# iqbal-lab-org/gramtools

Measured on AMD Instinct MI355X. Metric: 150bp reads quasimapped/sec (whole node); bit-exact coverage, higher is better.
Workload: dtype u32

## Files before the change

### gramtools_amd/_lib.py

```python
import ctypes as C
import os

from .build import LIB, build_library


class GmxError(RuntimeError):
    def __init__(self, code, msg):
        super().__init__(f"gmx error {code}: {msg}")
        self.code = code


class IndexInfo(C.Structure):
    _fields_ = [("n_text", C.c_uint64), ("kmer_size", C.c_uint32), ("n_sites", C.c_uint32), ("is_nested", C.c_uint32),
                ("n_allele_slots", C.c_uint32), ("n_per_base_slots", C.c_uint32), ("n_grouped_slots", C.c_uint32),
                ("n_nodes", C.c_uint32), ("n_kmers_present", C.c_uint64), ("index_bytes", C.c_uint64),
                ("kmer_size2", C.c_uint32), ("n_inline_sites", C.c_uint32), ("seed_shift", C.c_uint32),
                ("n_jump_sites", C.c_uint32), ("n_seed_words", C.c_uint64)]


class EngineOpts(C.Structure):
    _fields_ = [("device", C.c_int), ("rng_mode", C.c_int), ("max_states", C.c_uint32),
                ("max_path_nodes", C.c_uint32), ("max_batch_reads", C.c_uint64), ("forward_only", C.c_int),
                ("huge_heap_bytes", C.c_uint64), ("log_cap_words", C.c_uint64)]


class Stats(C.Structure):
    _fields_ = [("all_reads_count", C.c_uint64), ("skipped_reads_count", C.c_uint64),
                ("missing_kmer_reads_count", C.c_uint64), ("no_extension_reads_count", C.c_uint64),
                ("exact_mapped_reads_count", C.c_uint64)]


class QueueCounts(C.Structure):
    _fields_ = [(n, C.c_uint64) for n in ("mapped", "alive", "dead", "overflow_probe", "overflow_extend", "big_mapped",
                                          "cover_general", "cover_mid", "cover_overflow", "seed_cursor", "huge_search",
                                          "inst_mapped", "huge_cover", "log_replays", "log_replayed_entries", "overflow_split")]


class StockReport(C.Structure):
    _fields_ = [(n, C.c_uint64) for n in ("kmers", "states", "kmer_mismatches", "kmers_missing_in_files", "duplicate_kmers",
                                          "mask_bits", "mask_mismatches", "cov_graph_state", "cov_graph_library_version",
                                          "cov_graph_sites", "fm_index_bytes")]


class Timing(C.Structure):
    _fields_ = [("search_ms", C.c_double), ("search_launches", C.c_uint64), ("cover_ms", C.c_double),
                ("cover_launches", C.c_uint64), ("reads", C.c_uint64), ("kernel_ms", C.c_double * 8),
                ("kernel_launches", C.c_uint64 * 8)]


class BgzfMember(C.Structure):
    _fields_ = [("offset", C.c_uint64), ("size", C.c_uint32), ("isize", C.c_uint32), ("crc32", C.c_uint32), ("reserved", C.c_uint32)]


class IngestResult(C.Structure):
    _fields_ = [("status", C.c_uint32), ("bad_member", C.c_uint32), ("n_reads", C.c_uint64), ("n_bases", C.c_uint64),
                ("n_pairs", C.c_uint64), ("uniform_len", C.c_uint32), ("any_skip", C.c_uint32), ("text_bytes", C.c_uint64),
                ("consumed_bytes", C.c_uint64), ("tail_bytes", C.c_uint64), ("sub_pairs", C.c_uint64 * 16),
                ("d_planes", C.c_void_p), ("d_offsets", C.c_void_p), ("d_skip", C.c_void_p)]


class DepthStats(C.Structure):
    _fields_ = [("mean_cov_depth", C.c_double), ("variance_cov_depth", C.c_double), ("num_sites_noCov", C.c_uint64),
                ("num_sites_total", C.c_uint64)]


class DeviceCoverage(C.Structure):
    _fields_ = [("allele_sum", C.c_void_p), ("n_allele_sum", C.c_uint64), ("per_base", C.c_void_p),
                ("n_per_base", C.c_uint64), ("grouped", C.c_void_p), ("n_grouped", C.c_uint64),
                ("stats", C.c_void_p), ("n_stats", C.c_uint64), ("fused", C.c_void_p), ("n_fused", C.c_uint64)]


_vp, _u64, _u32, _i64 = C.c_void_p, C.c_uint64, C.c_uint32, C.c_int64
_u8p, _u32p, _i32p, _u64p, _i64p = (C.POINTER(C.c_uint8), C.POINTER(C.c_uint32), C.POINTER(C.c_int32),
                                    C.POINTER(C.c_uint64), C.POINTER(C.c_int64))
SYMBOLS = {
    "gmx_last_error": (C.c_char_p, []),
    "gmx_index_build": (C.c_int, [_u32p, _u64, _u32, C.c_int, C.POINTER(_vp)]),
    "gmx_index_build_from_file": (C.c_int, [C.c_char_p, _u32, C.c_int, C.POINTER(_vp)]),
    "gmx_index_save": (C.c_int, [_vp, C.c_char_p]),
    "gmx_index_load": (C.c_int, [C.c_char_p, C.c_char_p, _u32, C.POINTER(_vp)]),
    "gmx_index_destroy": (None, [_vp]),
    "gmx_index_get_info": (C.c_int, [_vp, C.POINTER(IndexInfo)]),
    "gmx_index_site_layout": (C.c_int, [_vp, _u32p, _u32p, _u32p, _u32p, _i32p]),
    "gmx_index_per_base_layout": (_i64, [_vp, _u32p, _u64]),
    "gmx_index_allele_base_layout": (C.c_int, [_vp, _u32p, _u32p]),
    "gmx_compute_coverage_depth": (C.c_int, [_vp, _u32p, _u32p, _u32p, _u64, C.POINTER(DepthStats)]),
    "gmx_index_bubble_order": (C.c_int, [_vp, _u32p]),
    "gmx_debug_suffix_array_u16": (C.c_int, [C.POINTER(C.c_uint16), _u64, C.POINTER(C.c_uint16)]),
    "gmx_index_copy_sa": (C.c_int, [_vp, _u32p]),
    "gmx_index_copy_bwt": (C.c_int, [_vp, _u32p]),
    "gmx_index_rank": (_u32, [_vp, _u32, _u32]),
    "gmx_index_copy_pos_info": (C.c_int, [_vp, _i64p]),
    "gmx_index_copy_target_map": (_i64, [_vp, _i64p, _u64]),
    "gmx_index_seed_states": (_i64, [_vp, _u8p, _i64p, _u64]),
    "gmx_index_seed_states_k": (_i64, [_vp, _u8p, _u32, _i64p, _u64]),
    "gmx_index_jump_states": (_i64, [_vp, _u32, _u32, _i64p, _u64]),
    "gmx_engine_default_opts": (None, [C.POINTER(EngineOpts)]),
    "gmx_engine_create": (C.c_int, [_vp, C.POINTER(EngineOpts), C.POINTER(_vp)]),
    "gmx_engine_destroy": (None, [_vp]),
    "gmx_engine_reset": (C.c_int, [_vp]),
    "gmx_engine_reset_async": (C.c_int, [_vp, _vp]),
    "gmx_map_reads_host": (C.c_int, [_vp, _u8p, _u64p, _u32p, _u64]),
    "gmx_map_reads_device": (C.c_int, [_vp, _vp, _vp, _vp, _u64, _u64, _vp]),
    "gmx_map_reads_packed_host": (C.c_int, [_vp, _vp, _vp, _u32, _vp, _vp, _u64]),
    "gmx_engine_sync_uploads": (C.c_int, [_vp]),
    "gmx_engine_seeds_in_place": (C.c_int, [_vp, C.c_int]),
    "gmx_packed_pairs": (_u64, [_u64p, _u32, _u64]),
    "gmx_twobit_units": (_u64, [_u64p, _u32, _u64]),
    "gmx_pack_reads_2bit": (C.c_int, [_vp, _vp, _u32, _u64, _vp, _vp, C.c_int]),
    "gmx_map_reads_2bit_host": (C.c_int, [_vp, _vp, _vp, _u32, _vp, _vp, _u64]),
    "gmx_map_reads_packed_device": (C.c_int, [_vp, _vp, _vp, _u32, _vp, _vp, _u64]),
    "gmx_ingest_create": (C.c_int, [C.c_int, _u64, C.POINTER(_vp)]),
    "gmx_ingest_destroy": (None, [_vp]),
    "gmx_ingest_max_text": (_u64, [_vp]),
    "gmx_ingest_max_compressed": (_u64, [_vp]),
    "gmx_ingest_reset": (C.c_int, [_vp]),
    "gmx_ingest_set_format": (C.c_int, [_vp, C.c_int]),
    "gmx_ingest_set_bam_header": (C.c_int, [_vp, _u64]),
    "gmx_ingest_bam_rewalks": (_i64, [_vp]),
    "gmx_ingest_submit_bgzf": (C.c_int, [_vp, C.c_int, _vp, _u64, C.POINTER(BgzfMember), _u64, C.c_int]),
    "gmx_ingest_submit_text": (C.c_int, [_vp, C.c_int, _vp, _u64, C.c_int]),
    "gmx_ingest_submit_gzip": (C.c_int, [_vp, C.c_int, _vp, _u64, _u64, C.c_int]),
    "gmx_ingest_gzip_repairs": (_i64, [_vp]),
    "gmx_ingest_submit_text_deferred": (C.c_int, [_vp, C.c_int, _vp, _u64]),
    "gmx_ingest_max_members": (_u64, [_vp]),
    "gmx_ingest_wait": (C.c_int, [_vp, C.c_int, C.POINTER(IngestResult)]),
    "gmx_ingest_submit_bgzf_deferred": (C.c_int, [_vp, C.c_int, _vp, _u64, C.POINTER(BgzfMember), _u64]),
    "gmx_ingest_scan": (C.c_int, [_vp, C.c_int, _vp, _u64, C.c_int]),
    "gmx_ingest_fetch_tail": (_i64, [_vp, C.c_int, _vp, _u64]),
    "gmx_ingest_release_after": (C.c_int, [_vp, C.c_int, _vp]),
    "gmx_ingest_fetch_text": (_i64, [_vp, C.c_int, _vp, _u64]),
    "gmx_ingest_fetch_reads": (C.c_int, [_vp, C.c_int, _vp, _vp, _vp]),
    "gmx_pack_reads": (C.c_int, [_vp, _vp, _u32, _u64, _vp, _vp, C.c_int]),
    "gmx_engine_reserve": (C.c_int, [_vp, _u64, _u64]),
    "gmx_engine_reserve_packed": (C.c_int, [_vp, _u64, _u64]),
    "gmx_host_alloc": (_vp, [_u64]),
    "gmx_host_free": (None, [_vp]),
    "gmx_engine_sync": (C.c_int, [_vp]),
    "gmx_engine_enable_timing": (C.c_int, [_vp, C.c_int]),
    "gmx_engine_timing": (C.c_int, [_vp, C.POINTER(Timing)]),
    "gmx_engine_queue_counts": (C.c_int, [_vp, C.POINTER(QueueCounts)]),
    "gmx_stock_read_int_vector": (_i64, [C.c_char_p, _u32, _u64p, _u64, C.POINTER(C.c_uint32)]),
    "gmx_stock_write_int_vector": (C.c_int, [C.c_char_p, _u64p, _u64, _u32, C.c_int]),
    "gmx_index_write_stock_files": (C.c_int, [_vp, C.c_char_p]),
    "gmx_index_check_stock_files": (C.c_int, [_vp, C.c_char_p, C.POINTER(StockReport)]),
    "gmx_engine_second_stream": (_vp, [_vp]),
    "gmx_engine_debug_keep_states": (C.c_int, [_vp, C.c_int]),
    "gmx_debug_fail_alloc": (C.c_uint64, [C.c_int64]),
    "gmx_debug_final_states": (C.c_int, [_vp, _u64, _u32p, _u64, _u64p, C.POINTER(C.c_int)]),
    "gmx_debug_search": (C.c_int, [_vp, _u8p, _u32, C.c_int, _u32p, _u64, _u32, _u32, C.c_int, _u32p, _u64, _u64p]),
    "gmx_debug_encapsulate": (C.c_int, [_vp, _u32p, _u64, _u32p, _u64, _u64p, _u32p, _u64, _u64p]),
    "gmx_master_seeds": (C.c_int, [_u32, _u64p, _u64, _u32p]),
    "gmx_coverage_device": (C.c_int, [_vp, C.POINTER(DeviceCoverage)]),
    "gmx_coverage_reduce_begin": (C.c_int, [_vp, _vp]),
    "gmx_coverage_reduce_end": (C.c_int, [_vp, _vp]),
    "gmx_coverage_fetch": (C.c_int, [_vp, _u32p, _u32p, _u32p, C.POINTER(Stats)]),
    "gmx_coverage_fetch_grouped_log": (_i64, [_vp, _u32p, _u64]),
    "gmx_engine_record_outcomes": (C.c_int, [_vp, C.c_int]),
    "gmx_engine_outcome_count": (_i64, [_vp]),
    "gmx_engine_fetch_outcomes": (C.c_int, [_vp, _u64, _u64, _u8p]),
    "gmx_engine_record_positions": (C.c_int, [_vp, C.c_int]),
    "gmx_engine_position_count": (_i64, [_vp]),
    "gmx_engine_fetch_positions": (C.c_int, [_vp, _u64, _u64, _u32p]),
    "gmx_engine_record_strands": (C.c_int, [_vp, C.c_int]),
    "gmx_engine_set_max_candidates": (C.c_int, [_vp, C.c_uint32]),
    "gmx_engine_max_candidates": (C.c_uint32, [_vp]),
    "gmx_coverage_fetch_strand": (C.c_int, [_vp, C.c_int, _u32p, _u32p, _u32p]),
    "gmx_coverage_fetch_grouped_log_strand": (_i64, [_vp, C.c_int, _u32p, _u64]),
    "gmx_coverage_export_grouped_log": (_i64, [_vp, _u32p, _u64]),
    "gmx_coverage_import_grouped_log": (C.c_int, [_vp, _u32p, _u64, C.c_int]),
    "gmx_grouped_log_merge_gathered": (_i64, [_vp, _vp, C.c_int, _u64, _vp, _u64]),
# ... 66 lines not shown
```

### gramtools_amd/csrc/gmx_capi.cpp

```cpp
#include <atomic>
#include <algorithm>
#include <array>
#include <cmath>
#include <cstdlib>
#include <cstring>
#include <map>
#include <new>
#include <stdexcept>
#include <system_error>
#include <string>
#include <thread>
#include <vector>

#include "gmx_core.h"
#include "gmx_internal.h"

static std::atomic<uint64_t> g_index_serial{1};
struct gmx_index {
  gmx::HostIndex h;
  const uint64_t serial = g_index_serial.fetch_add(1);
};

static thread_local std::string g_error;
void gmx_set_error(const std::string &msg) noexcept {
// ... 320 lines not shown
      uint32_t nm = (1u << site.n_alleles) - 1u;
      for (uint32_t m = 0; m < nm; ++m) {
        uint32_t tot = grouped_raw[h.l_grouped_off[s] + m];
        if (!tot) continue;
        uint16_t c = (uint16_t)(tot & 0xFFFFu);
        for (uint32_t a = 0; a < site.n_alleles; ++a)
          if (((m + 1) >> a) & 1u) hap[s][(int32_t)a] = (uint16_t)(hap[s][(int32_t)a] + c);
      }
    }
    for (auto &e : logged[s])
      for (auto a : e.first) hap[s][a] = (uint16_t)(hap[s][a] + e.second);
  }
  auto max_hap = [&](size_t s) -> std::pair<int32_t, uint16_t> {
    std::pair<int32_t, uint16_t> best{0, 0};
    bool any = false;
    for (auto &e : hap[s])
      if (!any || e.second > best.second) {
        best = {e.first, e.second};
        any = true;
      }
    return best;
  };
  std::vector<double> coverages;
  double total = 0;
  uint64_t no_cov = 0;
  for (uint32_t s : bubble_order(h)) {
    const GmxSite &site = h.sites[s];
    if (site.parent_site != 0) continue;
    auto mx = max_hap(s);
    uint16_t allele_cov = mx.second;
    double sum = 0;
    uint64_t n_bases = 0;
    uint32_t cur = site.entry_node;
    size_t guard = 0;
    while (cur != site.exit_node) {
      if (++guard > h.nodes.size() + 8) {
        gmx_set_error("coverage graph walk does not terminate");
        return GMX_EINVAL;
      }
      const GmxNode &nd = h.nodes[cur];
      uint32_t ne = h.nodes[cur + 1].edge_begin - nd.edge_begin;
      if (ne > 1 && nd.seq_len == 0) {
        auto m2 = max_hap((nd.site - 5) / 2);
        if (m2.first < 0 || (uint32_t)m2.first >= ne) {
          gmx_set_error("haplogroup out of range");
          return GMX_EINVAL;
        }
        cur = h.edges[nd.edge_begin + (uint32_t)m2.first];
        continue;
      }
      if (nd.seq_len > 0 && nd.cov_off != GMX_NO_COV)
        for (uint32_t i = 0; i < nd.seq_len; ++i) {
          uint32_t v = per_base_raw[h.l_cov_off[cur] + i];
          sum += (double)(v > 65535u ? 65535u : v);
          ++n_bases;
        }
      cur = h.edges[nd.edge_begin];
    }
    double site_cov = n_bases ? sum / (double)n_bases : (double)allele_cov;
    total += site_cov;
    coverages.push_back(site_cov);
    if (allele_cov == 0) no_cov++;
  }
  double mean = total / (double)coverages.size();
  double tv = 0;
  for (double c : coverages) tv += std::pow(c - mean, 2);
  out->mean_cov_depth = mean;
  out->variance_cov_depth = tv / (double)coverages.size();
  out->num_sites_noCov = no_cov;
  out->num_sites_total = coverages.size();
  return GMX_OK;
} GMX_GUARD_INT("gmx_compute_coverage_depth")

int gmx_debug_suffix_array_u16(const uint16_t *text, uint64_t n, uint16_t *out) try {
  try {
    gmx::debug_suffix_array_u16(text, (size_t)n, out);
    return GMX_OK;
  } catch (std::exception const &ex) {
    gmx_set_error(ex.what());
    return GMX_EINVAL;
  }
} GMX_GUARD_INT("gmx_debug_suffix_array_u16")

int gmx_index_copy_sa(const gmx_index *ix, uint32_t *out) try {
  memcpy(out, ix->h.sa.data(), ix->h.sa.size() * 4);
  return GMX_OK;
} GMX_GUARD_INT("gmx_index_copy_sa")
int gmx_index_copy_bwt(const gmx_index *ix, uint32_t *out) try {
  if (ix->h.bwt.empty()) {
    gmx_set_error("this index was built without its introspection tables (GMX_INDEX_INTROSPECTION=1 keeps them)");
    return GMX_EINVAL;
  }
  memcpy(out, ix->h.bwt.data(), ix->h.bwt.size() * 4);
  return GMX_OK;
} GMX_GUARD_INT("gmx_index_copy_bwt")
uint32_t gmx_index_rank(const gmx_index *ix, uint32_t upper, uint32_t base) try {
  if (base < 1 || base > 4) return 0;
  GmxIndexView v = ix->h.view();
  return gmx_rank(v, upper, base);
} GMX_GUARD_ZERO("gmx_index_rank")
int gmx_index_copy_pos_info(const gmx_index *ix, int64_t *out) try {
  const auto &h = ix->h;
  if (h.pos_target.size() != h.prg.size()) {
    gmx_set_error("this index was built without its introspection tables (GMX_INDEX_INTROSPECTION=1 keeps them)");
    return GMX_EINVAL;
  }
  for (size_t p = 0; p < h.prg.size(); ++p) {
    const GmxNode &nd = h.nodes[h.pos_node[p]];
    out[5 * p + 0] = nd.site;
    out[5 * p + 1] = nd.allele;
    out[5 * p + 2] = h.prg[p] <= 4 ? (int64_t)p - nd.first_pos : 0;
    out[5 * p + 3] = h.pos_target[p].first;
    out[5 * p + 4] = h.pos_target[p].second;
  }
  return GMX_OK;
} GMX_GUARD_INT("gmx_index_copy_pos_info")
int64_t gmx_index_copy_target_map(const gmx_index *ix, int64_t *out, uint64_t cap) try {
  std::vector<int64_t> v{(int64_t)ix->h.target_map.size()};
  for (auto &e : ix->h.target_map) {
    v.push_back(e.first);
    v.push_back((int64_t)e.second.size());
    for (auto &t : e.second) {
      v.push_back(t.id);
      v.push_back(t.deletion_allele);
    }
  }
  if (v.size() > cap) return -(int64_t)v.size();
  std::copy(v.begin(), v.end(), out);
  return (int64_t)v.size();
} GMX_GUARD_INT("gmx_index_copy_target_map")
int64_t gmx_index_seed_states(const gmx_index *ix, const uint8_t *kmer, int64_t *out, uint64_t cap) try {
  return gmx_index_seed_states_k(ix, kmer, ix->h.kmer_size, out, cap);
} GMX_GUARD_INT("gmx_index_seed_states")
int64_t gmx_index_seed_states_k(const gmx_index *ix, const uint8_t *kmer, uint32_t len, int64_t *out, uint64_t cap) try {
  const auto &h = ix->h;
  if (len == 0 || (len != h.kmer_size && len != h.kmer_size2)) return GMX_EINVAL;
  uint32_t code = 0;
  for (uint32_t j = 0; j < len; ++j) {
    if (kmer[j] < 1 || kmer[j] > 4) return GMX_EINVAL;
    code |= (uint32_t)(kmer[j] - 1) << (2 * j);
  }
  auto v = gmx::seed_states_of(h, code, len != h.kmer_size);
  if (v.size() > cap) return -(int64_t)v.size();
  std::copy(v.begin(), v.end(), out);
  return (int64_t)v.size();
} GMX_GUARD_INT("gmx_index_seed_states_k")
int64_t gmx_index_jump_states(const gmx_index *ix, uint32_t lo, uint32_t hi, int64_t *out, uint64_t cap) try {
  const auto &h = ix->h;
  GmxIndexView v = h.view();
  ProbeCtx ctx;
  const GmxRankBlock b = v.blocks[lo >> GMX_BLK_SHIFT];
  gmx_marker_pass(v, lo, hi, GMX_NIL, GMX_NIL, b, ctx);
  std::vector<int64_t> r{(int64_t)ctx.n};
  for (uint32_t s = 0; s < ctx.n; ++s) {
    r.push_back(ctx.st[s].lo);
    r.push_back(ctx.st[s].hi);
    std::vector<std::pair<uint32_t, int32_t>> tmp;
    for (uint32_t x = ctx.st[s].tvd; x != GMX_NIL; x = ctx.arena[x].next) tmp.push_back({ctx.arena[x].site, ctx.arena[x].allele});
    r.push_back((int64_t)tmp.size());
    for (size_t i = tmp.size(); i-- > 0;) {
      r.push_back(tmp[i].first);
      r.push_back(tmp[i].second);
    }
    tmp.clear();
    for (uint32_t x = ctx.st[s].tvg; x != GMX_NIL; x = ctx.arena[x].next) tmp.push_back({ctx.arena[x].site, -1});
    r.push_back((int64_t)tmp.size());
// ... 231 lines not shown
```

### gramtools_amd/csrc/gmx_engine_cover_kernels.h

```cpp
#pragma once
struct CoverAcc {
  uint32_t *acc;
  uint32_t *log;
  uint32_t *log_cursor;
  uint32_t log_cap;
  uint32_t *scratch_big;
  uint32_t n_lanes_big;
  int rng_mode;
  uint32_t max_candidates;
  uint32_t log_sites;
  uint32_t *heap;
  uint64_t heap_words;
  const uint32_t *status;
  uint32_t n_tasks;
  unsigned long long *stats;
  uint32_t rev_off;
  __device__ __forceinline__ uint32_t off_of(uint32_t task) const { return (task & 1u) ? rev_off : 0u; }
};

#define GMX_LOG_PAD 0xFFFFFFFFu
#ifdef GMX_LOOP_STATS
__device__ unsigned long long gmx_cover_stats[6 * 16];
__device__ unsigned long long gmx_coop_stats[6 * 8];
extern "C" int gmx_debug_coop_stats(unsigned long long *out, int reset) {
// ... 787 lines not shown

template <bool NESTED>
__global__ void __launch_bounds__(GMX_BLOCK) gmx_cover_single_kernel(GmxIndexView ix, BatchView b, SearchOut o, CoverAcc acc) {
  const uint32_t region = blockIdx.x & (GMX_REGIONS - 1);
  const uint32_t n_mapped = o.counters[(16 + region) * GMX_CNT_STRIDE];
  const uint32_t m = (blockIdx.x / GMX_REGIONS) * GMX_BLOCK + threadIdx.x;
  if (m >= n_mapped) return;
  gmx_cover_single_rec<NESTED>(ix, o, acc, (size_t)region * o.region_cap + m, o.cover_general_list, 8u);
}

struct StageLds {
  uint32_t *w;
  __device__ __forceinline__ uint32_t cap() const { return GMX_STAGE_MAX; }
  __device__ __forceinline__ void put(uint32_t i, uint32_t v) { w[i * GMX_BLOCK] = v; }
  __device__ __forceinline__ uint32_t get(uint32_t i) const { return w[i * GMX_BLOCK]; }
};
#ifndef GMX_JUMP_MIN_BLOCKS
#define GMX_JUMP_MIN_BLOCKS 1
#endif
__global__ void __launch_bounds__(GMX_BLOCK, GMX_JUMP_MIN_BLOCKS) gmx_cover_jump_kernel(GmxIndexView ix, BatchView b, SearchOut o, CoverAcc acc) {
  const uint32_t region = blockIdx.x & (GMX_REGIONS - 1);
  const uint32_t n_mapped = o.counters[(16 + region) * GMX_CNT_STRIDE];
  const uint32_t m = (blockIdx.x / GMX_REGIONS) * GMX_BLOCK + threadIdx.x;
  if (m >= n_mapped) return;
  const size_t rec_idx = (size_t)region * o.region_cap + m;
  CompactEnv env;
  env.rec = o.cover_recs[rec_idx];
  env.acc = acc.acc;
  env.acc_off = acc.rev_off ? acc.off_of(o.cover_rec_task[rec_idx]) : 0u;
  env.log = nullptr;
  env.log_cursor = nullptr;
  env.log_cap = 0;
  env.log_sites = 0;
  env.status = GMX_TASK_MAPPED;
  env.log_at = env.log_end = 0;
  const uint32_t p = env.rec.p, tvd = env.n_trav() ? 0u : GMX_NIL, tvg = env.rec.tvg;
  StageLds stage{gmx_lds + threadIdx.x};
  const bool done = gmx_cover_jump(ix, env, stage, p, tvd, tvg, env.rec.len_n & 0xFFFFu);
  if (!done) o.single_rest_list[atomicAdd(&o.counters[GMX_CNT_SINGLE_REST * GMX_CNT_STRIDE], 1u)] = (uint32_t)rec_idx;
}
__global__ void __launch_bounds__(GMX_BLOCK) gmx_cover_single_rest_kernel(GmxIndexView ix, BatchView b, SearchOut o, CoverAcc acc) {
  const uint32_t n = o.counters[GMX_CNT_SINGLE_REST * GMX_CNT_STRIDE];
  for (uint32_t i = blockIdx.x * GMX_BLOCK + threadIdx.x; i < n; i += gridDim.x * GMX_BLOCK)
    gmx_cover_single_rec<false>(ix, o, acc, o.single_rest_list[i], o.cover_general_list, 8u);
}

__global__ void gmx_log_replay_setup_kernel(SearchOut o, const uint32_t *retry_huge_in) {
  uint32_t *c = o.counters;
  const uint32_t n_entries = c[GMX_CNT_LOG_RETRY * GMX_CNT_STRIDE], n_recs = c[GMX_CNT_LOG_RETRY_RECS * GMX_CNT_STRIDE],
                 n_huge = c[GMX_CNT_LOG_RETRY_HUGE * GMX_CNT_STRIDE];
  for (uint32_t i = threadIdx.x; i < n_huge; i += blockDim.x) o.huge_list[i] = retry_huge_in[i];
  __syncthreads();
  if (threadIdx.x == 0) {
    c[4 * GMX_CNT_STRIDE] = n_entries;
    c[GMX_CNT_REPLAY_RECS * GMX_CNT_STRIDE] = n_recs;
    c[11 * GMX_CNT_STRIDE] = n_huge;
    c[15 * GMX_CNT_STRIDE] = 0;
    c[14 * GMX_CNT_STRIDE] = 0;
    c[GMX_CNT_LOG_RETRY * GMX_CNT_STRIDE] = 0;
    c[GMX_CNT_LOG_RETRY_RECS * GMX_CNT_STRIDE] = 0;
    c[GMX_CNT_LOG_RETRY_HUGE * GMX_CNT_STRIDE] = 0;
  }
}
template <bool NESTED>
__global__ void __launch_bounds__(GMX_BLOCK) gmx_cover_single_replay_kernel(GmxIndexView ix, BatchView b, SearchOut o, CoverAcc acc,
                                                                            const uint32_t *recs_in) {
  const uint32_t n = o.counters[GMX_CNT_REPLAY_RECS * GMX_CNT_STRIDE];
  for (uint32_t i = blockIdx.x * GMX_BLOCK + threadIdx.x; i < n; i += gridDim.x * GMX_BLOCK)
    gmx_cover_single_rec<NESTED>(ix, o, acc, recs_in[i], o.cover_overflow_list, 4u);
}

__global__ void gmx_stats_limbs_kernel(unsigned long long *stats, uint32_t *limbs, int recombine) {
  const uint32_t t = threadIdx.x;
  if (!recombine) {
    if (t < 20) limbs[t] = (uint32_t)((stats[t >> 2] >> (16 * (t & 3))) & 0xFFFFull);
    else if (t < 32) limbs[t] = 0;
  } else if (t < 5) {
    unsigned long long v = 0;
    for (int l = 3; l >= 0; --l) v = (v << 16) + limbs[4 * t + l];
    stats[t] = v;
  }
}

#define GMX_PACK_READS 128
#define GMX_PACK_IN_BYTES (24 * 1024)
#define GMX_PACK_OUT_PAIRS (GMX_PACK_IN_BYTES / 32 + GMX_PACK_READS + 8)
typedef uint32_t __attribute__((aligned(1))) gmx_u32_unaligned;
__device__ __forceinline__ void pack4(uint32_t x, uint32_t &lo, uint32_t &hi, uint32_t &bad) {
  uint32_t y = x - 0x01010101u;
  bad |= ((y & ~x & 0x80808080u) | (y & 0xFCFCFCFCu));
  lo = (((y & 0x01010101u) * 0x01020408u) >> 24) & 0xFu;
  hi = ((((y >> 1) & 0x01010101u) * 0x01020408u) >> 24) & 0xFu;
}
__device__ __forceinline__ uint2 pack_tail(const uint8_t *p, uint32_t rem, uint32_t &bad) {
  uint2 out = make_uint2(0, 0);
  for (uint32_t j = 0; j < rem; ++j) {
    uint32_t x = p[j];
    if (x < 1 || x > 4) bad = 1;
    out.x |= ((x - 1u) & 1u) << j;
    out.y |= (((x - 1u) >> 1) & 1u) << j;
  }
  return out;
}
#define GMX_PACK_THREADS (2 * GMX_PACK_READS)
__global__ void __launch_bounds__(GMX_PACK_THREADS) gmx_pack_kernel(BatchView b, uint8_t *skip, uint2 *packed, uint32_t *counters,
                                                                    uint32_t *zero, uint32_t zero_words) {
  __shared__ uint4 in4[GMX_PACK_IN_BYTES / 16 + 2];
  __shared__ uint2 outp[GMX_PACK_OUT_PAIRS];
  if (blockIdx.x == 0)
    for (uint32_t i = threadIdx.x; i < GMX_N_COUNTERS * GMX_CNT_STRIDE; i += GMX_PACK_THREADS) counters[i] = 0;
  for (uint32_t i = blockIdx.x * GMX_PACK_THREADS + threadIdx.x; i < zero_words; i += gridDim.x * GMX_PACK_THREADS) zero[i] = 0;
  const uint32_t r0 = blockIdx.x * GMX_PACK_READS;
  const uint32_t r1 = min(r0 + GMX_PACK_READS, b.n_reads);
  const uint32_t read = r0 + (threadIdx.x >> 1), half = threadIdx.x & 1u;
  const uint64_t s0 = b.offsets[r0], s1 = b.offsets[r1];
  const uintptr_t g0 = reinterpret_cast<uintptr_t>(b.reads + s0);
  const uint32_t shift = (uint32_t)(g0 & 15u);
  const uint64_t span = (s1 - s0) + shift;
  if (span <= GMX_PACK_IN_BYTES) {
    const uint4 *src = reinterpret_cast<const uint4 *>(g0 - shift);
    const uint32_t n16 = (uint32_t)((span + 15) >> 4);
    {
      uint32_t i = threadIdx.x;
      for (; i + 2 * GMX_PACK_THREADS < n16; i += 3 * GMX_PACK_THREADS) {
        const uint4 v0 = src[i], v1 = src[i + GMX_PACK_THREADS], v2 = src[i + 2 * GMX_PACK_THREADS];
        in4[i] = v0;
        in4[i + GMX_PACK_THREADS] = v1;
        in4[i + 2 * GMX_PACK_THREADS] = v2;
      }
      for (; i < n16; i += GMX_PACK_THREADS) in4[i] = src[i];
    }
    const uint64_t po0 = pack_off(b, r0);
    const uint32_t n_out = (uint32_t)(pack_off(b, r1) - po0);
    for (uint32_t i = threadIdx.x; i < n_out; i += GMX_PACK_THREADS) outp[i] = make_uint2(0, 0);
    __syncthreads();
    if (read < r1) {
      const uint64_t s = b.offsets[read];
      const uint32_t len = (uint32_t)(b.offsets[read + 1] - s);
      const uint32_t q = shift + (uint32_t)(s - s0);
      const uint32_t *w = reinterpret_cast<const uint32_t *>(in4);
      const uint8_t *bytes = reinterpret_cast<const uint8_t *>(in4);
      uint2 *out = outp + (uint32_t)(pack_off(b, read) - po0);
      const uint32_t full = len >> 5, first_half = (full + 1u) >> 1;
      const uint32_t c0 = half ? first_half : 0u, c1 = half ? full : first_half;
      uint32_t idx = (q >> 2) + 8u * c0;
      const uint32_t sh = q & 3u;
      uint32_t bad = 0;
      uint32_t carry = w[idx];
      for (uint32_t c = c0; c < c1; ++c) {
        uint2 pair = make_uint2(0, 0);
#pragma unroll
        for (int j = 0; j < 8; ++j) {
          uint32_t nxt = w[++idx], lo, hi;
          pack4(__builtin_amdgcn_alignbyte(nxt, carry, sh), lo, hi, bad);
          pair.x |= lo << (4 * j);
          pair.y |= hi << (4 * j);
          carry = nxt;
        }
        out[c] = pair;
      }
      const uint32_t rem = len & 31u;
      if (half && rem) out[full] = pack_tail(bytes + q + full * 32, rem, bad);
      bad |= (uint32_t)__shfl_xor((int)bad, 1);
      if (!half) skip[read] = bad ? 1 : 0;
    }
    __syncthreads();
// ... 26 lines not shown
```

### gramtools_amd/csrc/gmx_engine_debug.h

```cpp

struct GmxDebugPools {
  GmxFinalState *states = nullptr;
  uint32_t *stack = nullptr;
  GmxPathNode *arena = nullptr;
  uint32_t *result = nullptr;
  uint32_t *in = nullptr;
  uint2 *planes = nullptr;
  uint32_t cap_states = 0, cap_nodes = 0, cap_in = 0, cap_pairs = 0;
};

__global__ void __launch_bounds__(64) gmx_debug_search_kernel(GmxIndexView ix, BatchView b, const uint32_t *in, uint32_t from, uint32_t stop,
                                                              uint32_t mode, uint32_t from_seed_table, BigOut g, uint32_t *result) {
  const bool active = threadIdx.x == 0;
  BigCtx ctx;
  ctx.sp = 0;
  ctx.cap = g.max_states;
  ctx.stack = g.stack;
  ctx.arena = g.arena;
  ctx.arena_n = 0;
  ctx.arena_cap = g.max_path_nodes;
  ctx.status = GMX_TASK_MAPPED;
  ctx.out = g.states;
  ctx.n_out = 0;
  ctx.out_cap = g.max_states;
// ... 92 lines not shown
  for (uint32_t h = st.traversed; h != GMX_NIL;) {
    GmxPathNode nd;
    int rc = node(h, nd);
    if (rc) return rc;
    tvd.emplace_back(nd.site, nd.allele);
    h = nd.next;
    if (tvd.size() > (1u << 20)) {
      gmx_set_error("debug states: path list does not end");
      return GMX_EREF;
    }
  }
  for (uint32_t h = st.traversing; h != GMX_NIL;) {
    if (gmx_h_inline(h)) {
      tvg.push_back(5u + 2u * (h & ~GMX_INLINE_FLAG));
      break;
    }
    GmxPathNode nd;
    int rc = node(h, nd);
    if (rc) return rc;
    tvg.push_back(nd.site);
    h = nd.next;
    if (tvg.size() > (1u << 20)) {
      gmx_set_error("debug states: path list does not end");
      return GMX_EREF;
    }
  }
  w.put(lo);
  w.put(hi);
  w.put((uint32_t)tvd.size());
  w.put((uint32_t)tvg.size());
  for (size_t i = tvd.size(); i-- > 0;) {
    w.put(tvd[i].first);
    w.put((uint32_t)tvd[i].second);
  }
  for (size_t i = tvg.size(); i-- > 0;) w.put(tvg[i]);
  return GMX_OK;
}

int debug_pools(gmx_engine *e, GmxDebugPools &p, uint32_t n_in_words, uint32_t n_pairs) {
  const uint32_t S = std::max<uint32_t>(e->big.max_states, 64u), N = std::max<uint32_t>(e->big.max_path_nodes, 64u);
  int rc;
  if ((rc = e->alloc(&p.states, S, false))) return rc;
  if ((rc = e->alloc(&p.stack, (size_t)S * GMX_STACK_WORDS, false))) return rc;
  if ((rc = e->alloc(&p.arena, N, false))) return rc;
  if ((rc = e->alloc(&p.result, 4, true))) return rc;
  if ((rc = e->alloc(&p.in, std::max<uint32_t>(n_in_words, 1u), false))) return rc;
  if ((rc = e->alloc(&p.planes, n_pairs + 16, true))) return rc;
  p.cap_states = S;
  p.cap_nodes = N;
  return GMX_OK;
}
void debug_pools_free(gmx_engine *e, GmxDebugPools &p) {
  e->release(p.states);
  e->release(p.stack);
  e->release(p.arena);
  e->release(p.result);
  e->release(p.in);
  e->release(p.planes);
}

}

extern "C" {

int gmx_engine_debug_keep_states(gmx_engine *e, int on) try {
  if (!e) {
    gmx_set_error("null engine");
    return GMX_EINVAL;
  }
  e->keep_states = on != 0;
  return GMX_OK;
} GMX_GUARD_INT("gmx_engine_debug_keep_states")

int gmx_debug_final_states(gmx_engine *e, uint64_t task, uint32_t *out, uint64_t cap_words, uint64_t *n_words, int *tier) try {
  if (!e || !n_words) {
    gmx_set_error("gmx_debug_final_states: null argument");
    return GMX_EINVAL;
  }
  if (!e->keep_states || task >= 2 * e->keep_reads) {
    gmx_set_error("gmx_debug_final_states: no such task in the last batch (gmx_engine_debug_keep_states first)");
    return GMX_EINVAL;
  }
  HIP_TRY(hipSetDevice(e->opts.device));
  HIP_TRY(hipDeviceSynchronize());
  int rc = debug_isa(e);
  if (rc) return rc;
  uint32_t raw[GMX_N_COUNTERS * GMX_CNT_STRIDE];
  HIP_TRY(hipMemcpy(raw, e->d_counters, sizeof(raw), hipMemcpyDeviceToHost));
  auto c = [&](int i) { return raw[i * GMX_CNT_STRIDE]; };
  DebugWriter w{out, cap_words};
  {
    const uint32_t n_huge = c(11);
    std::vector<uint32_t> huge(n_huge);
    if (n_huge) HIP_TRY(hipMemcpy(huge.data(), e->d_huge, n_huge * sizeof(uint32_t), hipMemcpyDeviceToHost));
    for (uint32_t t : huge)
      if (t == task) {
        gmx_set_error("gmx_debug_final_states: the task was searched by the last tier, which keeps no states");
        return GMX_ECAP;
      }
  }
  const uint32_t used = (uint32_t)std::min<uint64_t>((uint64_t)c(1) + c(9) + c(29), e->big.max_slots);
  if (used) {
    std::vector<uint32_t> owner(used), nf(used), over(std::min<uint32_t>(c(1), used));
    HIP_TRY(hipMemcpy(owner.data(), e->big.task_of_slot, used * sizeof(uint32_t), hipMemcpyDeviceToHost));
    HIP_TRY(hipMemcpy(nf.data(), e->big.n_final, used * sizeof(uint32_t), hipMemcpyDeviceToHost));
    if (!over.empty()) HIP_TRY(hipMemcpy(over.data(), e->d_overflow, over.size() * sizeof(uint32_t), hipMemcpyDeviceToHost));
    bool in_slots = false;
    for (uint32_t s = used; s-- > 0;) {
      const bool first_q = s < over.size();
      if (first_q && (over[s] & ~GMX_INST_FLAG) != task) continue;
      if (!first_q && owner[s] != task) continue;
      in_slots = true;
      if (first_q && owner[s] != task) continue;
      if (nf[s] == 0) continue;
      const bool inst = first_q && (over[s] & GMX_INST_FLAG) != 0;
      const uint32_t n = nf[s];
      std::vector<GmxFinalState> st(n);
      if (inst) {
        uint32_t first = 0, width = 0;
        HIP_TRY(hipMemcpy(&first, e->d_inst_first + s, 4, hipMemcpyDeviceToHost));
        HIP_TRY(hipMemcpy(&width, e->d_inst_width + s, 4, hipMemcpyDeviceToHost));
        if (n > width * GMX_INST_STATES) continue;
        HIP_TRY(hipMemcpy(st.data(), e->d_inst_states + (size_t)first * GMX_INST_STATES, n * sizeof(GmxFinalState), hipMemcpyDeviceToHost));
        const GmxPathNode *arena = e->d_inst_arena + (size_t)first * GMX_FAST_ARENA;
        w.put(n);
        for (uint32_t i = 0; i < n; ++i) {
          rc = debug_put_state(e, w, st[i], [&](uint32_t h, GmxPathNode &nd) {
            HIP_TRY(hipMemcpy(&nd, arena + h, sizeof(nd), hipMemcpyDeviceToHost));
            return GMX_OK;
          });
          if (rc) return rc;
        }
        if (tier) *tier = 2;
      } else {
        if (n > e->big.max_states) continue;
        HIP_TRY(hipMemcpy(st.data(), e->big.states + (size_t)s * e->big.max_states, n * sizeof(GmxFinalState), hipMemcpyDeviceToHost));
        const GmxPathNode *arena = e->big.arena + (size_t)s * e->big.max_path_nodes;
        w.put(n);
        for (uint32_t i = 0; i < n; ++i) {
          rc = debug_put_state(e, w, st[i], [&](uint32_t h, GmxPathNode &nd) {
            HIP_TRY(hipMemcpy(&nd, arena + h, sizeof(nd), hipMemcpyDeviceToHost));
            return GMX_OK;
          });
          if (rc) return rc;
        }
        if (tier) *tier = 1;
      }
      *n_words = w.n;
      return w.n > cap_words && out ? GMX_ECAP : GMX_OK;
    }
    if (in_slots) {
      w.put(0);
      if (tier) *tier = 1;
      *n_words = w.n;
      return GMX_OK;
    }
  }
  uint32_t packed = 0;
  HIP_TRY(hipMemcpy(&packed, e->d_n_final + task, 4, hipMemcpyDeviceToHost));
  const uint32_t n = std::min<uint32_t>(packed & 0xFFu, GMX_FAST_STATES);
  std::vector<GmxFinalState> st(n);
  if (n) HIP_TRY(hipMemcpy(st.data(), e->d_finals + (size_t)task * GMX_FAST_STATES, n * sizeof(GmxFinalState), hipMemcpyDeviceToHost));
  const GmxPathNode *arena = e->d_arena + task;
  w.put(n);
  for (uint32_t i = 0; i < n; ++i) {
    rc = debug_put_state(e, w, st[i], [&](uint32_t h, GmxPathNode &nd) {
      HIP_TRY(hipMemcpy(&nd, arena + h, sizeof(nd), hipMemcpyDeviceToHost));
      return GMX_OK;
    });
    if (rc) return rc;
  }
  if (tier) *tier = 0;
  *n_words = w.n;
  return w.n > cap_words && out ? GMX_ECAP : GMX_OK;
} GMX_GUARD_INT("gmx_debug_final_states")

int gmx_debug_search(gmx_engine *e, const uint8_t *read, uint32_t read_len, int from_seed_table, const uint32_t *states, uint64_t n_state_words,
                     uint32_t from, uint32_t stop, int lf_only, uint32_t *out, uint64_t cap_words, uint64_t *n_words) try {
  if (!e || !read || !n_words || read_len == 0 || (!from_seed_table && (!states || n_state_words == 0 || from > read_len || stop > from))) {
    gmx_set_error("gmx_debug_search: bad argument");
    return GMX_EINVAL;
  }
  for (uint32_t i = 0; i < read_len; ++i)
    if (read[i] < 1 || read[i] > 4) {
      gmx_set_error("gmx_debug_search: the read must hold bases 1..4");
      return GMX_EINVAL;
    }
  if (from_seed_table && read_len < e->dview.kmer_size) {
    gmx_set_error("gmx_debug_search: read shorter than the k-mer size");
    return GMX_EINVAL;
  }
  HIP_TRY(hipSetDevice(e->opts.device));
  HIP_TRY(hipDeviceSynchronize());
  int rc = debug_isa(e);
  if (rc) return rc;
  const uint32_t n_pairs = (read_len + 31u) / 32u;
  GmxDebugPools p;
  if ((rc = debug_pools(e, p, (uint32_t)n_state_words, n_pairs))) return rc;
  std::vector<uint2> planes(n_pairs + 16, make_uint2(0, 0));
  for (uint32_t i = 0; i < read_len; ++i) {
    const uint32_t code = read[i] - 1u;
    planes[i >> 5].x |= (code & 1u) << (i & 31u);
    planes[i >> 5].y |= (code >> 1) << (i & 31u);
  }
  HIP_TRY(hipMemcpy(p.planes, planes.data(), planes.size() * sizeof(uint2), hipMemcpyHostToDevice));
  if (!from_seed_table) HIP_TRY(hipMemcpy(p.in, states, n_state_words * sizeof(uint32_t), hipMemcpyHostToDevice));
  BatchView b{};
  b.packed = p.planes;
  b.n_reads = 1;
  b.forward_only = 1;
  b.uniform_len = read_len;
  b.pairs_per_read = n_pairs;
  BigOut g{};
  g.states = p.states;
  g.stack = p.stack;
  g.arena = p.arena;
  g.max_states = p.cap_states;
  g.max_path_nodes = p.cap_nodes;
  g.max_slots = 1;
  const size_t big_lds = (size_t)GMX_BIG_LDS_DEPTH * GMX_STACK_WORDS * 64 * sizeof(uint32_t);
  hipLaunchKernelGGL(gmx_debug_search_kernel, dim3(1), dim3(64), big_lds, 0, e->dview, b, p.in, from, stop,
                     lf_only ? GMX_MODE_LF : GMX_MODE_STATE, from_seed_table ? 1u : 0u, g, p.result);
  HIP_TRY(hipGetLastError());
  HIP_TRY(hipDeviceSynchronize());
  uint32_t res[3] = {0, 0, 0};
  HIP_TRY(hipMemcpy(res, p.result, sizeof(res), hipMemcpyDeviceToHost));
  if (res[0] != GMX_TASK_MAPPED) {
    debug_pools_free(e, p);
    gmx_set_error(res[0] == GMX_TASK_OVERFLOW ? "gmx_debug_search: the states exceed the engine's large-capacity pools (gmx_engine_opts.max_states / max_path_nodes)"
                                              : "gmx_debug_search: the search reports a condition on which the reference throws");
    return res[0] == GMX_TASK_OVERFLOW ? GMX_ECAP : GMX_EREF;
  }
  const uint32_t n = res[1];
  std::vector<GmxFinalState> st(n);
  std::vector<GmxPathNode> arena(res[2]);
  if (n) HIP_TRY(hipMemcpy(st.data(), p.states, n * sizeof(GmxFinalState), hipMemcpyDeviceToHost));
  if (res[2]) HIP_TRY(hipMemcpy(arena.data(), p.arena, res[2] * sizeof(GmxPathNode), hipMemcpyDeviceToHost));
  debug_pools_free(e, p);
  DebugWriter w{out, cap_words};
  w.put(n);
  for (uint32_t i = 0; i < n; ++i) {
    rc = debug_put_state(e, w, st[i], [&](uint32_t h, GmxPathNode &nd) {
      if (h >= arena.size()) {
        gmx_set_error("gmx_debug_search: path handle outside the arena");
        return GMX_EREF;
      }
      nd = arena[h];
      return GMX_OK;
    });
    if (rc) return rc;
  }
  *n_words = w.n;
  return w.n > cap_words && out ? GMX_ECAP : GMX_OK;
} GMX_GUARD_INT("gmx_debug_search")

int gmx_debug_encapsulate(gmx_engine *e, const uint32_t *states, uint64_t n_state_words, uint32_t *out, uint64_t cap_words, uint64_t *n_words,
                          uint32_t *nonvariant_sa, uint64_t cap_nonvariant, uint64_t *n_nonvariant) try {
  if (!e || !states || n_state_words == 0 || !n_words || !n_nonvariant) {
    gmx_set_error("gmx_debug_encapsulate: bad argument");
    return GMX_EINVAL;
  }
  HIP_TRY(hipSetDevice(e->opts.device));
  HIP_TRY(hipDeviceSynchronize());
  std::vector<GmxFinalState> st;
  std::vector<GmxPathNode> arena;
  const uint32_t *p = states, *end = states + n_state_words;
  const uint32_t ns = *p++;
  uint64_t positions = 0;
  for (uint32_t s = 0; s < ns; ++s) {
    if (p + 4 > end || p + 4 + 2 * (uint64_t)p[2] + p[3] > end) {
      gmx_set_error("gmx_debug_encapsulate: malformed state words");
      return GMX_EINVAL;
    }
    const uint32_t lo = p[0], hi = p[1], nt = p[2], ng = p[3];
    p += 4;
    if (lo > hi || hi >= e->dview.n) {
      gmx_set_error("gmx_debug_encapsulate: interval outside the suffix array");
      return GMX_EINVAL;
    }
    uint32_t tvd = GMX_NIL, tvg = GMX_NIL;
    for (uint32_t j = 0; j < nt; ++j, p += 2) {
      arena.push_back(GmxPathNode{p[0], (int32_t)p[1], tvd});
      tvd = (uint32_t)arena.size() - 1;
    }
    for (uint32_t j = 0; j < ng; ++j, ++p) {
      arena.push_back(GmxPathNode{p[0], -1, tvg});
      tvg = (uint32_t)arena.size() - 1;
    }
    st.push_back(GmxFinalState{lo, hi, tvd, tvg});
    positions += (uint64_t)hi - lo + 1;
  }
  if (positions > (1u << 24)) {
    gmx_set_error("gmx_debug_encapsulate: more than 2^24 positions");
    return GMX_EINVAL;
  }
  const uint32_t cap_items = (uint32_t)std::max<uint64_t>(positions + ns, 1);
  GmxFinalState *d_st = nullptr;
  uint32_t *d_out = nullptr;
  int rc;
  if ((rc = e->alloc(&d_st, st.size(), false))) return rc;
  if ((rc = e->alloc(&d_out, 2 + 7 * (size_t)cap_items, true))) return rc;
  if (!st.empty()) HIP_TRY(hipMemcpy(d_st, st.data(), st.size() * sizeof(GmxFinalState), hipMemcpyHostToDevice));
  hipLaunchKernelGGL(gmx_debug_items_kernel, dim3(1), dim3(64), 0, 0, e->dview, d_st, (uint32_t)st.size(), d_out, cap_items);
  HIP_TRY(hipGetLastError());
  HIP_TRY(hipDeviceSynchronize());
  std::vector<uint32_t> res(2 + 7 * (size_t)cap_items);
  HIP_TRY(hipMemcpy(res.data(), d_out, res.size() * sizeof(uint32_t), hipMemcpyDeviceToHost));
  e->release(d_st);
  e->release(d_out);
  if (res[0] == 0xFFFFFFFFu || res[1] > cap_items) {
    gmx_set_error("gmx_debug_encapsulate: item buffer exceeded");
    return GMX_EREF;
  }
  DebugWriter w{out, cap_words};
  w.put(res[0]);
  for (uint32_t i = 0; i < res[0]; ++i) {
    const uint32_t *it = res.data() + 2 + 6 * (size_t)i;
    GmxFinalState f{it[0], it[1], it[2], it[3]};
    if (it[4] != 0) {
      w.put(f.lo);
      w.put(f.lo);
      w.put(1);
      w.put(0);
      w.put(it[4]);
      w.put(it[5]);
      continue;
    }
    rc = debug_put_state(e, w, f, [&](uint32_t h, GmxPathNode &nd) {
      if (h >= arena.size()) {
        gmx_set_error("gmx_debug_encapsulate: path handle outside the arena");
        return GMX_EREF;
      }
      nd = arena[h];
      return GMX_OK;
    });
    if (rc) return rc;
  }
  *n_words = w.n;
  *n_nonvariant = res[1];
  for (uint32_t i = 0; i < res[1] && nonvariant_sa && i < cap_nonvariant; ++i) nonvariant_sa[i] = res[2 + 6 * (size_t)cap_items + i];
  return (w.n > cap_words && out) || (nonvariant_sa && res[1] > cap_nonvariant) ? GMX_ECAP : GMX_OK;
} GMX_GUARD_INT("gmx_debug_encapsulate")

}
```

### gramtools_amd/csrc/gmx_engine_host.h

```cpp
#pragma once
#define HIP_TRY(expr)                                                                      \
  do {                                                                                     \
    hipError_t _e = (expr);                                                                \
    if (_e != hipSuccess) {                                                                \
      gmx_set_error(std::string(#expr) + ": " + hipGetErrorString(_e));                    \
      return GMX_EHIP;                                                                     \
    }                                                                                      \
  } while (0)

enum : int { GMX_TK_SEED = 0, GMX_TK_FILTER0, GMX_TK_FILTER1, GMX_TK_SINGLE, GMX_TK_EXTEND2, GMX_TK_UNPACK, GMX_TK_N };
static_assert(GMX_TK_N <= GMX_TIMED_KERNELS, "gmx_timing::kernel_ms holds GMX_TIMED_KERNELS entries");

struct GmxReadLog {
  const uint32_t stride;
  bool on = false;
  uint32_t *d = nullptr;
  uint64_t cap = 0, count = 0;

  uint64_t used() const { return (count * stride + 3) & ~3ull; }

  int reserve(uint64_t n_more) {
    const uint64_t need = (count + n_more) * stride;
    if (need <= cap) return GMX_OK;
    const uint64_t grown = (std::max<uint64_t>(need + need / 2, 1u << 20) + 3) & ~3ull;
// ... 72 lines not shown
  GmxFinalState *d_inst_states = nullptr;
  uint32_t *d_inst_first = nullptr, *d_inst_width = nullptr;
  uint32_t *d_inst_serial = nullptr, *d_general_serial = nullptr, *d_big_serial = nullptr, *d_overflow3 = nullptr;
  bool coop = true;
  uint32_t *d_heap = nullptr;
  uint64_t heap_words = 0;
  bool log_sites = false;
  std::map<std::vector<uint32_t>, std::array<uint64_t, 2>> log_counts;
  uint32_t *h_log_state = nullptr;
  hipEvent_t ev_log_state = nullptr;
  bool log_state_pending = false;
  uint32_t *d_log_retry[2] = {nullptr, nullptr}, *d_log_retry_recs[2] = {nullptr, nullptr}, *d_log_retry_huge[2] = {nullptr, nullptr};
  int log_retry_side = 0;
  BatchView last_b{};
  SearchOut last_o{};
  CoverAcc last_acc{};
  size_t last_big_lds = 0;
  uint64_t log_replays = 0, log_replayed_entries = 0;
  uint64_t log_known = 0;
  uint64_t log_reads_since = 0;
  bool reset_pending = false;
  hipStream_t reset_stream = nullptr;
  hipStream_t side2_stream = nullptr;
  hipEvent_t ev_fork2 = nullptr, ev_side1 = nullptr, ev_filter = nullptr;
  hipStream_t side_stream = nullptr;
  hipEvent_t ev_fork = nullptr, ev_join = nullptr;
  hipEvent_t ev_wait = nullptr;
  struct GmxDeviceIndex *shared_index = nullptr;
  uint32_t filter_lds_words = 0;
  const uint32_t *d_kmer_planar = nullptr;
  const uint32_t *d_absent = nullptr;
  uint32_t n_absent = 0;
  bool use_absent = false;
  uint32_t n_cus = 256;
  uint32_t probe_iters = GMX_PROBE_ITERS;
  uint32_t extend_cap = 0;
  uint32_t extend_budget = 8;
  bool seeds_in_place = false;
  gmx_engine *twin = nullptr;
  gmx_engine *owner = nullptr;
  bool is_twin = false, twin_off = false;
  GmxReadLog outcomes{1}, positions{16};
  uint64_t reset_epoch = 0;
  hipStream_t main_stream = nullptr;
  uint32_t twin_toggle = 0;
  hipEvent_t ev_zeroed = nullptr, ev_twin_done = nullptr;
  uint64_t zero_epoch = 0, seen_zero_epoch = 0;
  bool twin_in_flight = false;
  bool last_on_twin = false;
  uint32_t extend_passes = 1;
  uint32_t extend_budget2[GMX_EXTRA_PASSES] = {24, 96, 0};
  GmxParked *d_park2 = nullptr;
  uint32_t *d_park2_n = nullptr;
  bool keep_states = false;
  uint64_t keep_reads = 0;
  std::vector<uint32_t> debug_isa;
  uint32_t fuse = 1;
  uint8_t *d_reads = nullptr;
  uint64_t *d_offsets = nullptr;
  uint32_t *d_seeds = nullptr;
  uint64_t cap_bases = 0, cap_stage_reads = 0;
  struct StageSlot {
    uint8_t *d_reads = nullptr;
    uint64_t *d_offsets = nullptr, *h_offsets = nullptr;
    uint32_t *d_seeds = nullptr, *h_seeds = nullptr;
    uint64_t cap_bases = 0, cap_reads = 0;
    hipEvent_t copied = nullptr, done = nullptr;
    bool busy = false;
  } stage[2];
  hipStream_t copy_stream = nullptr;
  hipStream_t copy_stream2 = nullptr;
  uint32_t copy_toggle = 0;
  hipStream_t last_stream = nullptr;
  struct PackSlot {
    uint2 *d_planes = nullptr;
    uint64_t *d_offsets = nullptr;
    uint32_t *d_seeds = nullptr;
    uint8_t *d_skip = nullptr;
    uint64_t cap_pairs = 0, cap_reads = 0;
    hipEvent_t copied = nullptr, done = nullptr;
    bool busy = false;
  } pslot[3];
  uint32_t pslot_next = 0;
  void release(void *q) {
    if (!q) return;
    for (size_t i = 0; i < allocs.size(); ++i)
      if (allocs[i] == q) {
        allocs[i] = allocs.back();
        allocs.pop_back();
        (void)hipFree(q);
        return;
      }
  }
  bool timing = false;
  struct EvTriple { hipEvent_t s, a, b, c; uint64_t reads; hipEvent_t k[GMX_TIMED_KERNELS][2]; uint32_t timed; };
  std::vector<EvTriple> pending;
  double search_ms = 0, cover_ms = 0;
  uint64_t search_launches = 0, cover_launches = 0, timed_reads = 0;
  double kernel_ms[GMX_TIMED_KERNELS] = {0};
  uint64_t kernel_launches[GMX_TIMED_KERNELS] = {0};

  template <class T>
  int alloc(T **p, size_t count, bool zero) {
    void *q = nullptr;
    size_t bytes = std::max<size_t>(count, 1) * sizeof(T);
    allocs.reserve(allocs.size() + 1);
    HIP_TRY(hipMalloc(&q, bytes));
    if (zero) HIP_TRY(hipMemset(q, 0, bytes));
    allocs.push_back(q);
    *p = (T *)q;
    return GMX_OK;
  }
  template <class T, class A>
  int upload(const T **dst, const std::vector<T, A> &src) {
    T *q = nullptr;
    int rc = alloc(&q, src.size(), false);
    if (rc) return rc;
    if (!src.empty()) HIP_TRY(hipMemcpy(q, src.data(), src.size() * sizeof(T), hipMemcpyHostToDevice));
    index_bytes += src.size() * sizeof(T);
    *dst = q;
    return GMX_OK;
  }
  int upload(const uint32_t **dst, const gmx::WordBuf &src) {
    uint32_t *q = nullptr;
    int rc = alloc(&q, src.size(), false);
    if (rc) return rc;
    const size_t piece = (size_t)1 << 28;
    for (size_t at = 0; at < src.size(); at += piece)
      HIP_TRY(hipMemcpy(q + at, src.data() + at, std::min(piece, src.size() - at) * sizeof(uint32_t), hipMemcpyHostToDevice));
    index_bytes += src.size() * sizeof(uint32_t);
    *dst = q;
    return GMX_OK;
  }
};

static hipError_t gmx_event_wait(hipEvent_t ev) {
  static const bool spin = getenv("GMX_WAIT_SPIN") != nullptr;
  if (spin) return hipEventSynchronize(ev);
  const auto t0 = std::chrono::steady_clock::now();
  for (bool napping = false;;) {
    const hipError_t q = hipEventQuery(ev);
    if (q != hipErrorNotReady) return q;
    (void)hipGetLastError();
    if (!napping) {
      napping = std::chrono::steady_clock::now() - t0 > std::chrono::microseconds(60);
      continue;
    }
    struct timespec ts = {0, 50 * 1000};
    nanosleep(&ts, nullptr);
  }
}

static int gmx_quiesce(gmx_engine *e) {
  if (!e->ev_wait) HIP_TRY(hipEventCreateWithFlags(&e->ev_wait, hipEventDisableTiming | hipEventBlockingSync));
  hipStream_t streams[5] = {e->last_stream, e->copy_stream, e->side_stream, e->side2_stream, e->copy_stream2};
  for (int i = 0; i < 5; ++i) {
    if (i > 0 && !streams[i]) continue;
    bool seen = false;
    for (int j = 0; j < i; ++j) seen = seen || streams[j] == streams[i];
    if (seen) continue;
    HIP_TRY(hipEventRecord(e->ev_wait, streams[i]));
    HIP_TRY(gmx_event_wait(e->ev_wait));
  }
  return GMX_OK;
}

static int note_zeroed(gmx_engine *e, hipStream_t stream) {
  if (!e->twin) return GMX_OK;
  if (!e->ev_zeroed) HIP_TRY(hipEventCreateWithFlags(&e->ev_zeroed, hipEventDisableTiming));
  HIP_TRY(hipEventRecord(e->ev_zeroed, stream));
  ++e->zero_epoch;
  return GMX_OK;
}
static int twin_join(gmx_engine *e, hipStream_t stream) {
  gmx_engine *tw = e->twin;
  if (!tw || !e->twin_in_flight) return GMX_OK;
  if (!e->ev_twin_done) HIP_TRY(hipEventCreateWithFlags(&e->ev_twin_done, hipEventDisableTiming));
  HIP_TRY(hipEventRecord(e->ev_twin_done, tw->main_stream));
  HIP_TRY(hipStreamWaitEvent(stream, e->ev_twin_done, 0));
  return GMX_OK;
}
static int flush_reset(gmx_engine *e) {
  if (!e->reset_pending) return GMX_OK;
  e->reset_pending = false;
  HIP_TRY(hipMemsetAsync(e->d_fused, 0, (e->n_fused + 32) * 4, e->reset_stream));
  return note_zeroed(e, e->reset_stream);
}

static int log_settle(gmx_engine *e);
static int gmx_log_drain(gmx_engine *e, uint64_t keep_below) {
  int frc = flush_reset(e);
  if (frc) return frc;
  HIP_TRY(hipDeviceSynchronize());
  uint32_t used = 0;
  HIP_TRY(hipMemcpy(&used, e->d_log_cursor, 4, hipMemcpyDeviceToHost));
  used = std::min(used, e->log_cap);
  e->log_reads_since = 0;
  e->log_known = used;
  if (used <= keep_below) return GMX_OK;
  std::vector<uint32_t> w(used);
  HIP_TRY(hipMemcpy(w.data(), e->d_log, (size_t)used * 4, hipMemcpyDeviceToHost));
  std::vector<uint32_t> key;
  for (size_t i = 0; i < w.size();) {
    if (w[i] == GMX_LOG_PAD) {
      ++i;
      continue;
    }
    const size_t n_ids = i + 2 > w.size() ? 0 : (size_t)(w[i + 1] & ~GMX_LOG_REVERSE);
    if (i + 2 > w.size() || i + 2 + n_ids > w.size()) {
      gmx_set_error("grouped-allele-count log: malformed record at word " + std::to_string(i) + " of " + std::to_string(w.size()));
      return GMX_EREF;
    }
    if ((w[i + 1] & GMX_LOG_REVERSE) && !(e->owner ? e->owner : e)->record_strands) {
      gmx_set_error("grouped-allele-count log: a reverse-complement record at word " + std::to_string(i) + " of an engine that does not record per strand");
      return GMX_EREF;
    }
    key.assign(1, w[i]);
    key.insert(key.end(), w.begin() + i + 2, w.begin() + i + 2 + n_ids);
    e->log_counts[key][(w[i + 1] & GMX_LOG_REVERSE) ? 1 : 0] += 1;
    i += 2 + n_ids;
  }
  HIP_TRY(hipMemset(e->d_log_cursor, 0, 4));
  e->log_known = 0;
  return GMX_OK;
}

template <class Env, int LIST>
static void launch_cover_lds(gmx_engine *e, hipStream_t stream, const BatchView &b, const SearchOut &o, const CoverAcc &acc,
                             bool after_coop = false) {
  static const uint32_t lanes_env = getenv("GMX_COVER_LANES") ? (uint32_t)atoi(getenv("GMX_COVER_LANES")) : 0u;
  const uint32_t lanes = lanes_env ? std::min(lanes_env, gmx_cover_lds_lanes<Env>()) : gmx_cover_lds_lanes<Env>();
  const size_t lds = (size_t)GmxScratchFixed<Env>::total * lanes * sizeof(uint32_t);
  const uint32_t per_cu = std::min<uint32_t>((uint32_t)(160 * 1024 / lds), 32u);
  hipLaunchKernelGGL((gmx_cover_kernel<Env, LIST>), dim3(e->n_cus * per_cu), dim3(64), lds, stream, e->dview, b, o, e->big,
                     acc, lanes, after_coop ? 1u : 0u);
}

template <int LIST>
static void launch_cover_coop(gmx_engine *e, hipStream_t stream, const BatchView &b, const SearchOut &o, const CoverAcc &acc) {
  const size_t lds = (size_t)gmx_coop_lds_words<LIST>() * sizeof(uint32_t);
  const uint32_t per_cu = std::min<uint32_t>((uint32_t)(160 * 1024 / lds), 16u);
  hipLaunchKernelGGL((gmx_cover_coop_kernel<LIST>), dim3(e->n_cus * per_cu), dim3(64), lds, stream, e->dview, b, o, e->big, acc);
}

extern "C" {

void gmx_engine_default_opts(gmx_engine_opts *o) try {
  o->device = 0;
  o->rng_mode = GMX_RNG_LEMIRE;
  o->max_states = 1024;
  o->max_path_nodes = 2048;
  o->max_batch_reads = 4u << 20;
  o->forward_only = 0;
  o->huge_heap_bytes = 512ull << 20;
  o->log_cap_words = 0;
} GMX_GUARD_VOID("gmx_engine_default_opts")

static int ensure_batch_capacity(gmx_engine *e, uint64_t n_reads, bool launching = false) {
  if (launching) {
    gmx_engine *own = e->owner ? e->owner : e;
    for (GmxReadLog *log : {&own->outcomes, &own->positions})
      if (log->on) {
        const int lrc = log->reserve(n_reads);
        if (lrc) return lrc;
      }
  }
  if (n_reads <= e->cap_reads) return GMX_OK;
  uint64_t cap = std::max<uint64_t>(e->cap_reads ? n_reads + n_reads / 8 : n_reads, 1024);
  uint64_t n_tasks = cap * 2;
  int rc;
  if ((rc = e->alloc(&e->d_skip, cap, true))) return rc;
  if ((rc = e->alloc(&e->d_status, n_tasks, false))) return rc;
  if ((rc = e->alloc(&e->d_n_final, n_tasks, false))) return rc;
  if ((rc = e->alloc(&e->d_cover_recs, n_tasks * GMX_REGIONS, false))) return rc;
  if ((rc = e->alloc(&e->d_mapped, n_tasks * GMX_REGIONS, false))) return rc;
  if ((rc = e->alloc(&e->d_task_lists, (size_t)GMX_TL_N * n_tasks, false))) return rc;
  e->d_overflow = e->d_task_lists + (size_t)GMX_TL_OVERFLOW * n_tasks;
  e->d_overflow2 = e->d_task_lists + (size_t)GMX_TL_OVERFLOW2 * n_tasks;
  e->d_alive = e->d_task_lists + (size_t)GMX_TL_ALIVE * n_tasks;
  e->d_dead = e->d_task_lists + (size_t)GMX_TL_DEAD * n_tasks;
  e->d_dead2 = e->d_task_lists + (size_t)GMX_TL_DEAD2 * n_tasks;
  e->d_cover_general = e->d_task_lists + (size_t)GMX_TL_GENERAL * n_tasks;
  if ((rc = e->alloc(&e->d_cover_overflow, n_tasks, false))) return rc;
  if ((rc = e->alloc(&e->d_general_rest, n_tasks, false))) return rc;
  if ((rc = e->alloc(&e->d_single_rest, n_tasks, false))) return rc;
  if ((rc = e->alloc(&e->d_park2, (size_t)n_tasks * GMX_STACK_DEPTH, false))) return rc;
  if ((rc = e->alloc(&e->d_park2_n, n_tasks, false))) return rc;
  if (e->log_sites)
    for (int side = 0; side < 2; ++side) {
      if ((rc = e->alloc(&e->d_log_retry[side], n_tasks, false))) return rc;
      if ((rc = e->alloc(&e->d_log_retry_recs[side], n_tasks, false))) return rc;
      if ((rc = e->alloc(&e->d_log_retry_huge[side], n_tasks, false))) return rc;
    }
  if ((rc = e->alloc(&e->d_cover_mid, n_tasks, false))) return rc;
  if ((rc = e->alloc(&e->d_seed_cursor, n_tasks, false))) return rc;
  if ((rc = e->alloc(&e->d_finals, n_tasks * GMX_FAST_STATES, false))) return rc;
  if ((rc = e->alloc(&e->d_arena, n_tasks * GMX_FAST_ARENA, false))) return rc;
  if ((rc = e->alloc(&e->d_alive_seed, n_tasks, false))) return rc;
  if ((rc = e->alloc(&e->d_huge, n_tasks, false))) return rc;
  if ((rc = e->alloc(&e->d_cover_huge, n_tasks, false))) return rc;
  if ((rc = e->alloc(&e->d_huge_retry, 2 * n_tasks, false))) return rc;
  e->big.max_slots = (uint32_t)std::min<uint64_t>(n_tasks, std::min<uint64_t>(std::max<uint64_t>(n_tasks / 16, 4096), 262144));
  if ((rc = e->alloc(&e->big.states, (size_t)e->big.max_slots * e->big.max_states, false))) return rc;
  if ((rc = e->alloc(&e->big.stack, (size_t)e->big.max_slots * e->big.max_states * GMX_STACK_WORDS, false))) return rc;
  if ((rc = e->alloc(&e->big.arena, (size_t)e->big.max_slots * e->big.max_path_nodes, false))) return rc;
  if ((rc = e->alloc(&e->big.n_final, e->big.max_slots, false))) return rc;
  if ((rc = e->alloc(&e->big.task_of_slot, e->big.max_slots, false))) return rc;
  if ((rc = e->alloc(&e->d_big_mapped, e->big.max_slots, false))) return rc;
  e->inst_cap = (uint32_t)std::min<uint64_t>(n_tasks, 1u << 23);
  if ((rc = e->alloc(&e->d_inst_list, e->inst_cap, false))) return rc;
  if ((rc = e->alloc(&e->d_inst_sa, e->inst_cap, false))) return rc;
  if ((rc = e->alloc(&e->d_inst_remaining, e->big.max_slots, false))) return rc;
  if ((rc = e->alloc(&e->d_inst_mapped, e->big.max_slots, false))) return rc;
  if ((rc = e->alloc(&e->d_inst_first, e->big.max_slots, false))) return rc;
  if ((rc = e->alloc(&e->d_inst_width, e->big.max_slots, false))) return rc;
  if ((rc = e->alloc(&e->d_inst_serial, e->big.max_slots, false))) return rc;
  if ((rc = e->alloc(&e->d_general_serial, n_tasks, false))) return rc;
  if ((rc = e->alloc(&e->d_big_serial, e->big.max_slots, false))) return rc;
  if ((rc = e->alloc(&e->d_overflow3, 2 * n_tasks, false))) return rc;
  if ((rc = e->alloc(&e->d_inst_arena, (size_t)e->inst_cap * GMX_FAST_ARENA, false))) return rc;
  if ((rc = e->alloc(&e->d_inst_states, (size_t)e->inst_cap * GMX_INST_STATES, false))) return rc;
  e->cap_reads = cap;
  return GMX_OK;
}

struct GmxDeviceIndex {
  uint64_t serial = 0;
  int device = 0;
  GmxIndexView view{};
  std::vector<void *> allocs;
  uint64_t bytes = 0;
  int refs = 0;
};
static std::mutex g_dev_index_mu;
static std::vector<GmxDeviceIndex *> g_dev_indexes;
static void gmx_dev_index_release(GmxDeviceIndex *d) {
  if (!d) return;
  std::lock_guard<std::mutex> lk(g_dev_index_mu);
  if (--d->refs > 0) return;
  for (void *p : d->allocs) (void)hipFree(p);
  g_dev_indexes.erase(std::remove(g_dev_indexes.begin(), g_dev_indexes.end(), d), g_dev_indexes.end());
// ... 153 lines not shown
                   : e->log_sites     ? (1ull << 26)
                                      : 64;
    e->log_cap = (uint32_t)std::min<uint64_t>(cap, 0xFFFFFF00ull);
  }
  if (primary)
    e->d_log = primary->d_log;
  else
    rc |= e->alloc(&e->d_log, e->log_cap, false);
  e->heap_words = opts.huge_heap_bytes / 4 / 64 * 64;
  rc |= e->alloc(&e->d_heap, e->heap_words, false);
  rc |= e->alloc(&e->d_counters, GMX_N_COUNTERS * GMX_CNT_STRIDE, true);
  e->big.max_states = opts.max_states;
  e->big.max_path_nodes = opts.max_path_nodes;
  e->big.max_slots = 0;
  {
    hipDeviceProp_t prop;
    if (hipGetDeviceProperties(&prop, opts.device) == hipSuccess && prop.multiProcessorCount > 0)
      e->n_cus = (uint32_t)prop.multiProcessorCount;
    const size_t words = h.kmer_bitmap.size();
    if (!getenv("GMX_FORCE_ABSENT_FILTER") && words >= 4 && words % 4 == 0 && words * 4 <= 128 * 1024 &&
        hipFuncSetAttribute(reinterpret_cast<const void *>(gmx_filter_lds_kernel), hipFuncAttributeMaxDynamicSharedMemorySize,
                            (int)(words * 4)) == hipSuccess)
      e->filter_lds_words = (uint32_t)words;
    (void)hipGetLastError();
    if (primary) {
      e->filter_lds_words = primary->filter_lds_words;
      e->d_kmer_planar = primary->d_kmer_planar;
      e->d_absent = primary->d_absent;
      e->n_absent = primary->n_absent;
      e->use_absent = primary->use_absent;
    } else if (e->filter_lds_words) {
      const uint32_t k = h.kmer_size;
      std::vector<uint32_t> planar(words, 0);
      for (uint64_t code = 0; code < (1ull << (2 * k)); ++code) {
        if (!((h.kmer_bitmap[code >> 5] >> (code & 31)) & 1u)) continue;
        uint32_t lo = 0, hi = 0;
        for (uint32_t j = 0; j < k; ++j) {
          const uint32_t base = (uint32_t)(code >> (2 * j)) & 3u;
          lo |= (base & 1u) << j;
          hi |= (base >> 1) << j;
        }
        const uint32_t p = (hi << k) | lo;
        planar[p >> 5] |= 1u << (p & 31);
      }
      rc |= e->upload(&e->d_kmer_planar, planar);
    } else if (!getenv("GMX_NO_ABSENT_FILTER")) {
      const uint64_t n_k = 1ull << (2 * h.kmer_size);
      if (n_k - std::min<uint64_t>(n_k, h.n_seed_kmers_present) <= GMX_ABSENT_MAX) {
        std::vector<uint32_t> absent;
        for (size_t w = 0; w < words && absent.size() <= GMX_ABSENT_MAX; ++w) {
          uint32_t zeros = ~h.kmer_bitmap[w];
          while (zeros) {
            const uint64_t code = (uint64_t)w * 32 + (uint32_t)__builtin_ctz(zeros);
            zeros &= zeros - 1;
            if (code < n_k) absent.push_back((uint32_t)code);
          }
        }
        if (absent.size() <= GMX_ABSENT_MAX) {
          e->n_absent = (uint32_t)absent.size();
          e->use_absent = true;
          if (absent.empty()) absent.push_back(0);
          rc |= e->upload(&e->d_absent, absent);
        }
      }
    }
  }
  if (const char *pi = getenv("GMX_PROBE_ITERS")) e->probe_iters = (uint32_t)std::max(0, atoi(pi));
  if (getenv("GMX_NO_FUSE")) e->fuse = 0;
  if (const char *eb = getenv("GMX_EXTEND_BUDGET")) e->extend_budget = (uint32_t)std::max(0, atoi(eb));
  e->extend_cap = 0u;
  if (const char *ec = getenv("GMX_EXTEND_CAP")) e->extend_cap = (uint32_t)std::max(0, atoi(ec));
  e->extend_passes = 1u;
  e->extend_budget2[0] = 24;
  e->extend_budget2[1] = 96;
  if (const char *ep = getenv("GMX_EXTEND_PASSES")) {
    e->extend_passes = 1;
    for (const char *q = ep; *q && e->extend_passes < GMX_EXTRA_PASSES;) {
      e->extend_budget2[e->extend_passes - 1] = (uint32_t)std::max(1l, strtol(q, const_cast<char **>(&q), 10));
      ++e->extend_passes;
      if (*q == ',') ++q; else break;
    }
  }
  if (getenv("GMX_NO_COOP")) e->coop = false;
  e->seed_cursor = h.n_seed_states_large * 10 > h.n_seed_states;
  if (const char *sc = getenv("GMX_SEED_CURSOR")) e->seed_cursor = atoi(sc) != 0;
  if (primary) {
    e->seed_cursor = primary->seed_cursor;
    e->dview.sa_ctx = primary->dview.sa_ctx;
    e->dview.seed_side = primary->dview.seed_side;
  }
  if (!primary && e->seed_cursor && !rc && !getenv("GMX_NO_SA_CTX")) {
    uint32_t *sc = nullptr;
    if (e->alloc(&sc, h.sa.size(), false) == GMX_OK) {
      hipLaunchKernelGGL(gmx_sa_ctx_kernel, dim3(8192), dim3(256), 0, nullptr, e->dview.sa, e->dview.text, (uint64_t)h.sa.size(), sc);
      if (hipDeviceSynchronize() == hipSuccess) {
        e->dview.sa_ctx = sc;
        e->index_bytes += h.sa.size() * sizeof(uint32_t);
      }
    } else {
      (void)hipGetLastError();
    }
  }
  if (!primary && e->seed_cursor && !rc && !getenv("GMX_NO_SEED_SIDE") && h.seed_words.size() > 1) {
    uint32_t *side = nullptr;
    const size_t n_side = h.seed_words.size() / 4 + 2;
    if (e->alloc(&side, n_side, false) == GMX_OK) {
      hipLaunchKernelGGL(gmx_seed_side_kernel, dim3(8192), dim3(256), 0, nullptr, e->dview.seeds, (uint64_t)h.seeds.size(), e->dview.seed_words,
                         e->dview.seed_shift, side);
      if (h.kmer_size2)
        hipLaunchKernelGGL(gmx_seed_side_kernel, dim3(8192), dim3(256), 0, nullptr, e->dview.seeds2, (uint64_t)h.seeds2.size(), e->dview.seed_words,
                           e->dview.seed_shift, side);
      if (hipDeviceSynchronize() == hipSuccess) {
        e->dview.seed_side = side;
        e->index_bytes += n_side * sizeof(uint32_t);
      }
    } else {
      (void)hipGetLastError();
    }
  }
  auto make_stream = [&](hipStream_t *st) -> bool {
    int least = 0, greatest = 0;
    bool want_prio = h.is_nested;
    if (const char *tp = getenv("GMX_TWIN_PRIORITY")) want_prio = atoi(tp) != 0;
    const bool prio = primary && want_prio && hipDeviceGetStreamPriorityRange(&least, &greatest) == hipSuccess && least != greatest;
    (void)hipGetLastError();
    return (prio ? hipStreamCreateWithPriority(st, hipStreamNonBlocking, greatest) : hipStreamCreateWithFlags(st, hipStreamNonBlocking)) == hipSuccess;
  };
  rc |= !make_stream(&e->side_stream);
  rc |= !make_stream(&e->side2_stream);
  rc |= hipEventCreateWithFlags(&e->ev_fork2, hipEventDisableTiming) != hipSuccess;
  rc |= hipEventCreateWithFlags(&e->ev_side1, hipEventDisableTiming) != hipSuccess;
  rc |= hipEventCreateWithFlags(&e->ev_filter, hipEventDisableTiming) != hipSuccess;
  rc |= hipEventCreateWithFlags(&e->ev_fork, hipEventDisableTiming) != hipSuccess;
  rc |= hipEventCreateWithFlags(&e->ev_join, hipEventDisableTiming) != hipSuccess;
  e->cover_big_lanes = 64 * 32;
  rc |= e->alloc(&e->d_scratch_big, (size_t)GmxScratchFixed<CoverEnvBig>::total * e->cover_big_lanes, false);
  if (primary) {
    e->is_twin = true;
    rc |= !make_stream(&e->main_stream);
    e->last_stream = e->main_stream;
  }
  if (rc) {
    gmx_engine_destroy(e);
    return GMX_EHIP;
  }
  *out = e;
  return GMX_OK;
}

void gmx_engine_destroy(gmx_engine *e) try {
  if (!e) return;
  (void)hipSetDevice(e->opts.device);
  (void)hipDeviceSynchronize();
  if (e->twin) gmx_engine_destroy(e->twin);
  e->twin = nullptr;
  if (e->main_stream) (void)hipStreamDestroy(e->main_stream);
  if (e->ev_zeroed) (void)hipEventDestroy(e->ev_zeroed);
  if (e->ev_twin_done) (void)hipEventDestroy(e->ev_twin_done);
  if (e->side_stream) (void)hipStreamDestroy(e->side_stream);
  if (e->side2_stream) (void)hipStreamDestroy(e->side2_stream);
  if (e->ev_fork2) (void)hipEventDestroy(e->ev_fork2);
  if (e->ev_side1) (void)hipEventDestroy(e->ev_side1);
  if (e->ev_filter) (void)hipEventDestroy(e->ev_filter);
  if (e->ev_fork) (void)hipEventDestroy(e->ev_fork);
  if (e->ev_join) (void)hipEventDestroy(e->ev_join);
  if (e->ev_wait) (void)hipEventDestroy(e->ev_wait);
  if (e->copy_stream) (void)hipStreamDestroy(e->copy_stream);
  if (e->copy_stream2) (void)hipStreamDestroy(e->copy_stream2);
  if (e->h_log_state) (void)hipHostFree(e->h_log_state);
  if (e->ev_log_state) (void)hipEventDestroy(e->ev_log_state);
  for (auto &sl : e->pslot) {
    if (sl.copied) (void)hipEventDestroy(sl.copied);
    if (sl.done) (void)hipEventDestroy(sl.done);
  }
  for (auto &sl : e->stage) {
    if (sl.copied) (void)hipEventDestroy(sl.copied);
    if (sl.done) (void)hipEventDestroy(sl.done);
    if (sl.h_offsets) (void)hipHostFree(sl.h_offsets);
    if (sl.h_seeds) (void)hipHostFree(sl.h_seeds);
  }
  for (void *p : e->allocs) (void)hipFree(p);
  e->outcomes.release();
  e->positions.release();
  gmx_dev_index_release(e->shared_index);
  delete e;
} GMX_GUARD_VOID("gmx_engine_destroy")

int gmx_engine_reset(gmx_engine *e) try {
  HIP_TRY(hipSetDevice(e->opts.device));
  e->reset_pending = false;
  HIP_TRY(hipDeviceSynchronize());
  HIP_TRY(hipMemset(e->d_fused, 0, (e->n_fused + 32) * 4));
  HIP_TRY(hipMemset(e->d_error, 0, 8));
  HIP_TRY(hipMemset(e->d_counters, 0, GMX_N_COUNTERS * GMX_CNT_STRIDE * 4));
  if (e->twin) {
    HIP_TRY(hipMemset(e->twin->d_error, 0, 8));
    HIP_TRY(hipMemset(e->twin->d_counters, 0, GMX_N_COUNTERS * GMX_CNT_STRIDE * 4));
    e->twin_in_flight = false;
  }
  int lrc = e->outcomes.clear(nullptr);
  if (lrc || (lrc = e->positions.clear(nullptr))) return lrc;
  ++e->reset_epoch;
  e->log_counts.clear();
  e->log_known = e->log_reads_since = 0;
  e->log_state_pending = false;
  e->recorded = false;
  return GMX_OK;
} GMX_GUARD_INT("gmx_engine_reset")

int gmx_engine_reset_async(gmx_engine *e, void *hip_stream) try {
  HIP_TRY(hipSetDevice(e->opts.device));
  hipStream_t st = (hipStream_t)hip_stream;
  int frc = flush_reset(e);
  if (frc) return frc;
  if ((frc = twin_join(e, st))) return frc;
  e->twin_in_flight = false;
  if ((frc = e->outcomes.clear(&st)) || (frc = e->positions.clear(&st))) return frc;
  ++e->reset_epoch;
  e->reset_pending = true;
  e->reset_stream = st;
  e->log_counts.clear();
  e->log_known = e->log_reads_since = 0;
  e->log_state_pending = false;
  e->recorded = false;
  return GMX_OK;
} GMX_GUARD_INT("gmx_engine_reset_async")

static bool gmx_ab_no_filter() {
  static const bool off = getenv("GMX_AB_NO_FILTER") != nullptr;
  return off;
}
static void launch_filter(gmx_engine *e, hipStream_t st, dim3 task_grid, const BatchView &b, const SearchOut &o, int pass,
                          hipEvent_t t0 = nullptr, hipEvent_t t1 = nullptr) {
  if (gmx_ab_no_filter()) return;
  if (e->filter_lds_words)
    hipExtLaunchKernelGGL(gmx_filter_lds_kernel, dim3(e->n_cus), dim3(GMX_FILTER_LDS_THREADS), e->filter_lds_words * 4,
                          st, t0, t1, 0u, e->dview, b, o, e->d_kmer_planar, e->filter_lds_words, pass);
  else if (e->use_absent)
    hipExtLaunchKernelGGL(gmx_filter_absent_kernel, task_grid, dim3(GMX_BLOCK), 0, st, t0, t1, 0u, e->dview, b, o, e->d_absent, e->n_absent, pass);
  else
    hipExtLaunchKernelGGL(gmx_filter_kernel, task_grid, dim3(GMX_BLOCK), 0, st, t0, t1, 0u, e->dview, b, o, pass);
}

static int log_state_enqueue(gmx_engine *e, hipStream_t stream) {
  if (!e->h_log_state) {
    HIP_TRY(hipHostMalloc(reinterpret_cast<void **>(&e->h_log_state), 4 * sizeof(uint32_t), hipHostMallocDefault));
    HIP_TRY(hipEventCreateWithFlags(&e->ev_log_state, hipEventDisableTiming));
  }
  HIP_TRY(hipMemcpyAsync(e->h_log_state + 0, e->d_log_cursor, 4, hipMemcpyDeviceToHost, stream));
  HIP_TRY(hipMemcpyAsync(e->h_log_state + 1, e->d_counters + GMX_CNT_LOG_RETRY * GMX_CNT_STRIDE, 4, hipMemcpyDeviceToHost, stream));
  HIP_TRY(hipMemcpyAsync(e->h_log_state + 2, e->d_counters + GMX_CNT_LOG_RETRY_RECS * GMX_CNT_STRIDE, 4, hipMemcpyDeviceToHost, stream));
  HIP_TRY(hipMemcpyAsync(e->h_log_state + 3, e->d_counters + GMX_CNT_LOG_RETRY_HUGE * GMX_CNT_STRIDE, 4, hipMemcpyDeviceToHost, stream));
  HIP_TRY(hipEventRecord(e->ev_log_state, stream));
  e->log_state_pending = true;
  return GMX_OK;
}

static int launch_log_replay(gmx_engine *e, hipStream_t stream) {
  const int in = e->log_retry_side, out = in ^ 1;
  SearchOut o = e->last_o;
  o.log_retry_list = e->d_log_retry[out];
  o.log_retry_recs = e->d_log_retry_recs[out];
  o.log_retry_huge = e->d_log_retry_huge[out];
  o.cover_overflow_list = e->d_log_retry[in];
  hipLaunchKernelGGL(gmx_log_replay_setup_kernel, dim3(1), dim3(1024), 0, stream, o, e->d_log_retry_huge[in]);
  if (e->dview.is_nested)
    hipLaunchKernelGGL(gmx_cover_single_replay_kernel<true>, dim3(e->n_cus * 4), dim3(GMX_BLOCK), 0, stream, e->dview, e->last_b, o, e->last_acc,
                     e->d_log_retry_recs[in]);
  else
    hipLaunchKernelGGL(gmx_cover_single_replay_kernel<false>, dim3(e->n_cus * 4), dim3(GMX_BLOCK), 0, stream, e->dview, e->last_b, o, e->last_acc,
                     e->d_log_retry_recs[in]);
  hipLaunchKernelGGL((gmx_cover_kernel<CoverEnvBig, 1>), dim3(e->cover_big_lanes / 64), dim3(64), e->last_big_lds, stream, e->dview,
                     e->last_b, o, e->big, e->last_acc, 64u, 0u);
  HIP_TRY(hipGetLastError());
  e->log_retry_side = out;
  e->last_o.log_retry_list = o.log_retry_list;
  e->last_o.log_retry_recs = o.log_retry_recs;
  e->last_o.log_retry_huge = o.log_retry_huge;
  return log_state_enqueue(e, stream);
}

static int log_settle(gmx_engine *e) {
  if (!e->log_state_pending) return GMX_OK;
  uint64_t before = ~0ull;
  for (int round = 0;; ++round) {
    HIP_TRY(hipEventSynchronize(e->ev_log_state));
    e->log_state_pending = false;
    const uint32_t used = std::min(e->h_log_state[0], e->log_cap);
    const uint64_t retries = (uint64_t)e->h_log_state[1] + e->h_log_state[2] + e->h_log_state[3];
    if (retries == 0) {
      if (used > e->log_cap / 2) return gmx_log_drain(e, 0);
      e->log_known = used;
      return GMX_OK;
    }
    if (round > 0 && retries >= before) {
      HIP_TRY(hipDeviceSynchronize());
      const uint32_t err[2] = {GMX_TASK_LOGFULL, 0};
      HIP_TRY(hipMemcpy(e->d_error, err, 8, hipMemcpyHostToDevice));
      return GMX_OK;
    }
    before = retries;
    int rc = gmx_log_drain(e, 0);
    if (rc) return rc;
    e->log_replays++;
    e->log_replayed_entries += retries;
    if ((rc = launch_log_replay(e, e->last_stream))) return rc;
  }
}

struct BatchInput {
  const uint8_t *d_reads = nullptr;
  const uint64_t *d_offsets = nullptr;
  const uint32_t *d_seeds = nullptr;
  const uint2 *d_planes = nullptr;
  const uint8_t *d_skip = nullptr;
  const uint32_t *d_twobit = nullptr;
  uint32_t twobit_base0 = 0;
  uint32_t uniform_len = 0;
  uint64_t n_reads = 0, total_bases = 0;
};

__global__ void gmx_batch_begin_kernel(uint32_t *counters, uint32_t *zero, uint32_t zero_words) {
  if (blockIdx.x == 0)
    for (uint32_t i = threadIdx.x; i < GMX_N_COUNTERS * GMX_CNT_STRIDE; i += blockDim.x) counters[i] = 0;
  for (uint32_t i = blockIdx.x * blockDim.x + threadIdx.x; i < zero_words; i += gridDim.x * blockDim.x) zero[i] = 0;
}

__device__ __forceinline__ uint32_t gmx_even_bits(unsigned long long x) {
  x &= 0x5555555555555555ull;
  x = (x | (x >> 1)) & 0x3333333333333333ull;
  x = (x | (x >> 2)) & 0x0F0F0F0F0F0F0F0Full;
  x = (x | (x >> 4)) & 0x00FF00FF00FF00FFull;
  x = (x | (x >> 8)) & 0x0000FFFF0000FFFFull;
  x = (x | (x >> 16)) & 0x00000000FFFFFFFFull;
  return (uint32_t)x;
}
__global__ void __launch_bounds__(256) gmx_unpack2_kernel(BatchView b, const uint32_t *stream, uint32_t base0, uint2 *packed) {
  const uint32_t ppr_uniform = b.pairs_per_read;
  for (uint64_t t = blockIdx.x * (uint64_t)blockDim.x + threadIdx.x;; t += (uint64_t)gridDim.x * blockDim.x) {
    uint32_t read, pair;
    uint64_t first_base;
    uint32_t len;
    if (b.uniform_len) {
      read = (uint32_t)(t / ppr_uniform);
      if (read >= b.n_reads) break;
      pair = (uint32_t)(t - (uint64_t)read * ppr_uniform);
      first_base = (uint64_t)read * b.uniform_len;
      len = b.uniform_len;
    } else {
      read = (uint32_t)t;
      if (read >= b.n_reads) break;
      pair = 0;
      first_base = b.offsets[read] - b.offsets[0];
      len = (uint32_t)(b.offsets[read + 1] - b.offsets[read]);
    }
    uint2 *out = packed + pack_off(b, read);
    const uint32_t n_pairs = b.uniform_len ? pair + 1 : (len + 31u) / 32u;
    for (uint32_t p = pair; p < n_pairs; ++p) {
      const uint64_t j = base0 + first_base + 32ull * p;
      const uint64_t w = j >> 4;
      const uint32_t sh = (uint32_t)(j & 15u) * 2u;
      const uint32_t w0 = stream[w], w1 = stream[w + 1], w2 = stream[w + 2];
      const unsigned long long bits = (unsigned long long)__builtin_amdgcn_alignbit(w1, w0, sh) |
                                      ((unsigned long long)__builtin_amdgcn_alignbit(w2, w1, sh) << 32);
      out[p] = make_uint2(gmx_even_bits(bits), gmx_even_bits(bits >> 1));
    }
  }
}

static int launch_batch(gmx_engine *e, const BatchInput &in, hipStream_t stream) {
  const uint64_t n_reads = in.n_reads, total_bases = in.total_bases;
  if (n_reads == 0) return GMX_OK;
  if (n_reads > (0x7fffffffull / GMX_FAST_ARENA) / 2) {
    gmx_set_error("batch too large: at most 44 M reads per launch (lower gmx_engine_opts.max_batch_reads)");
    return GMX_EINVAL;
  }
  int rc = e->log_sites ? log_settle(e) : GMX_OK;
  if (rc) return rc;
  if ((rc = ensure_batch_capacity(e, n_reads, true))) return rc;
  const bool fold_reset = e->reset_pending && e->reset_stream == stream;
  if (e->reset_pending && !fold_reset && (rc = flush_reset(e))) return rc;
  e->reset_pending = false;
  if (!in.d_planes) {
    uint64_t need = total_bases / 32 + n_reads + 16;
    if (need > e->cap_packed) {
      rc = e->alloc(&e->d_packed, need, false);
      if (rc) return rc;
      e->cap_packed = need;
    }
  }
  BatchView b{in.d_reads, in.d_offsets, in.d_seeds, (in.d_planes || in.d_twobit) ? in.d_skip : e->d_skip, in.d_planes ? in.d_planes : e->d_packed,
              (uint32_t)n_reads, (uint32_t)(e->opts.forward_only ? 1 : 0), in.uniform_len, (in.uniform_len + 31u) / 32u,
              e->keep_states ? 1u : 0u};
  const uint32_t region_inv = (uint32_t)std::min<uint64_t>(0xFFFFFFFFull, (((uint64_t)GMX_REGIONS << 32) + e->dview.n_prg - 1) / std::max<uint32_t>(e->dview.n_prg, 1u));
  SearchOut o{};
  o.status = e->d_status;
  o.n_final = e->d_n_final;
  o.finals = e->d_finals;
  o.arena = e->d_arena;
  o.cover_recs = e->d_cover_recs;
  o.cover_rec_task = e->d_mapped;
  o.region_cap = (uint32_t)(e->cap_reads * 2);
  o.region_inv = region_inv;
  o.task_lists = e->d_task_lists;
  o.list_stride = (uint32_t)(e->cap_reads * 2);
  o.overflow_list = e->d_overflow;
  o.overflow2_list = e->d_overflow2;
  o.cover_overflow_list = e->d_cover_overflow;
  o.big_mapped_list = e->d_big_mapped;
  o.cover_mid_list = e->d_cover_mid;
  o.cover_general_list = e->d_cover_general;
  o.alive_list = e->d_alive;
  o.dead_list = e->d_dead;
  o.dead2_list = e->d_dead2;
  o.seed_cursor = e->d_seed_cursor;
  o.error = e->d_error;
  o.counters = e->d_counters;
  o.alive_seed = e->d_alive_seed;
  o.huge_list = e->d_huge;
  o.cover_huge_list = e->d_cover_huge;
  o.huge_retry = e->d_huge_retry;
  o.arena_stride = (uint32_t)(e->cap_reads * 2);
  o.inst_list = e->d_inst_list;
  o.inst_sa = e->d_inst_sa;
  o.inst_remaining = e->d_inst_remaining;
  o.inst_cap = e->inst_cap;
  o.inst_slots = !getenv("GMX_NO_INST") ? e->big.max_slots : 0u;
  o.slot_n_final = e->big.n_final;
  o.slot_task = e->big.task_of_slot;
  o.inst_mapped_list = e->d_inst_mapped;
  o.inst_arena = e->d_inst_arena;
  o.inst_states = e->d_inst_states;
  o.inst_first = e->d_inst_first;
  o.inst_remaining_width = e->d_inst_width;
  o.inst_serial_list = e->d_inst_serial;
  o.general_serial_list = e->d_general_serial;
  o.big_serial_list = e->d_big_serial;
  o.overflow3_list = e->d_overflow3;
  o.split_twice = getenv("GMX_NO_SPLIT2") ? 0u : 1u;
  o.general_rest_list = e->d_general_rest;
  o.single_rest_list = e->d_single_rest;
  o.park2 = e->d_park2;
  o.park2_n = e->d_park2_n;
  o.log_retry_list = e->d_log_retry[e->log_retry_side];
  o.log_retry_recs = e->d_log_retry_recs[e->log_retry_side];
  o.log_retry_huge = e->d_log_retry_huge[e->log_retry_side];
  o.stats = e->d_stats;
  {
    gmx_engine *own = e->owner ? e->owner : e;
    own->recorded = true;
    if (own->outcomes.on) {
      o.outcomes = own->outcomes.d;
      o.outcome_base = own->outcomes.claim(n_reads);
    }
    if (own->positions.on) {
// ... 111 lines not shown
    launch_cover_lds<CoverEnvLds, 3>(e, e->side_stream, b, o, acc, e->coop);
    launch_cover_lds<CoverEnv, 0>(e, e->side_stream, b, o, acc);
  }
  HIP_TRY(hipEventRecord(e->ev_filter, e->side_stream));
  if (e->dview.is_nested) {
    hipExtLaunchKernelGGL(gmx_cover_single_kernel<true>, dim3(task_grid.x * GMX_REGIONS), dim3(GMX_BLOCK), 0, stream, t_ev(GMX_TK_SINGLE, 0), t_ev(GMX_TK_SINGLE, 1), 0u,
                          e->dview, b, o, acc);
  } else if (e->cover_jump) {
    hipExtLaunchKernelGGL(gmx_cover_jump_kernel, dim3(task_grid.x * GMX_REGIONS), dim3(GMX_BLOCK), (uint32_t)(GMX_STAGE_MAX * GMX_BLOCK * sizeof(uint32_t)), stream,
                          t_ev(GMX_TK_SINGLE, 0), t_ev(GMX_TK_SINGLE, 1), 0u, e->dview, b, o, acc);
    hipLaunchKernelGGL(gmx_cover_single_rest_kernel, dim3(e->n_cus * 2), dim3(GMX_BLOCK), 0, stream, e->dview, b, o, acc);
  } else {
    hipExtLaunchKernelGGL(gmx_cover_single_kernel<false>, dim3(task_grid.x * GMX_REGIONS), dim3(GMX_BLOCK), 0, stream, t_ev(GMX_TK_SINGLE, 0), t_ev(GMX_TK_SINGLE, 1), 0u,
                          e->dview, b, o, acc);
  }
  hipStream_t last = general_on_side ? e->side2_stream : stream;
  if (!general_on_side) {
    launch_one(stream);
    if (e->coop) launch_cover_coop<3>(e, stream, b, o, acc);
    launch_cover_lds<CoverEnvLds, 3>(e, stream, b, o, acc, e->coop);
    launch_cover_lds<CoverEnv, 0>(e, stream, b, o, acc);
    HIP_TRY(hipEventRecord(e->ev_join, e->side2_stream));
    HIP_TRY(hipStreamWaitEvent(stream, e->ev_join, 0));
  }
  HIP_TRY(hipStreamWaitEvent(last, e->ev_filter, 0));
  hipLaunchKernelGGL((gmx_cover_kernel<CoverEnvBig, 1>), dim3(e->cover_big_lanes / 64), dim3(64), big_lds, last, e->dview,
                     b, o, e->big, acc, 64u, 0u);
  if (general_on_side) {
    HIP_TRY(hipEventRecord(e->ev_join, e->side2_stream));
    HIP_TRY(hipStreamWaitEvent(stream, e->ev_join, 0));
  }
  if (e->timing) {
    HIP_TRY(hipEventRecord(ev.c, stream));
    e->pending.push_back(ev);
  }
  HIP_TRY(hipGetLastError());
  e->last_stream = stream;
  if (e->log_sites) {
    e->last_b = b;
    e->last_o = o;
    e->last_acc = acc;
    e->last_big_lds = big_lds;
    if ((rc = log_state_enqueue(e, stream))) return rc;
  }
  return GMX_OK;
}

int gmx_map_reads_device(gmx_engine *e, const uint8_t *d_reads, const uint64_t *d_offsets, const uint32_t *d_seeds,
                         uint64_t n_reads, uint64_t total_bases, void *hip_stream) try {
  if (!e) {
    gmx_set_error("null engine");
    return GMX_EINVAL;
  }
  HIP_TRY(hipSetDevice(e->opts.device));
  hipStream_t stream = (hipStream_t)hip_stream;
  uint64_t done = 0;
  while (done < n_reads) {
    uint64_t n = std::min<uint64_t>(e->opts.max_batch_reads, n_reads - done);
    BatchInput in;
    in.d_reads = d_reads;
    in.d_offsets = d_offsets + done;
    in.d_seeds = d_seeds + done;
    in.n_reads = n;
    in.total_bases = total_bases;
    int rc = launch_batch(e, in, stream);
    if (rc) return rc;
    done += n;
  }
  if (e->log_sites) return log_settle(e);
  return GMX_OK;
} GMX_GUARD_INT("gmx_map_reads_device")

static bool gmx_is_pinned(const void *p) {
  hipPointerAttribute_t at;
  if (hipPointerGetAttributes(&at, p) != hipSuccess) {
    (void)hipGetLastError();
    return false;
  }
  return at.type == hipMemoryTypeHost;
}

static int map_reads_host_pipelined(gmx_engine *e, const uint8_t *reads, const uint64_t *offsets, const uint32_t *seeds,
                                    uint64_t n_reads, uint64_t chunk) {
  if (!e->copy_stream) HIP_TRY(hipStreamCreateWithFlags(&e->copy_stream, hipStreamNonBlocking));
  const uint64_t first = offsets[0], total = offsets[n_reads] - first;
  const bool registered = !gmx_is_pinned(reads + first) &&
                          hipHostRegister(const_cast<uint8_t *>(reads + first), total, hipHostRegisterDefault) == hipSuccess;
  (void)hipGetLastError();
  int rc = GMX_OK;
  auto hip_ok = [&](hipError_t err, const char *what) {
    if (err == hipSuccess) return true;
    gmx_set_error(std::string(what) + ": " + hipGetErrorString(err));
    rc = GMX_EHIP;
    return false;
  };
  uint64_t done = 0;
  try {
  for (uint32_t i = 0; done < n_reads && rc == GMX_OK; ++i) {
    gmx_engine::StageSlot &sl = e->stage[i & 1];
    const uint64_t n = std::min<uint64_t>(chunk, n_reads - done);
    const uint64_t b0 = offsets[done], bases = offsets[done + n] - b0;
    if (sl.busy) {
      if (!hip_ok(gmx_event_wait(sl.done), "hipEventSynchronize")) break;
      sl.busy = false;
    }
    if (!sl.copied) {
      if (!hip_ok(hipEventCreateWithFlags(&sl.copied, hipEventDisableTiming | hipEventBlockingSync), "hipEventCreate") ||
          !hip_ok(hipEventCreateWithFlags(&sl.done, hipEventDisableTiming | hipEventBlockingSync), "hipEventCreate"))
        break;
    }
    if (bases > sl.cap_bases) {
      const uint64_t cb = std::max<uint64_t>(bases + bases / 8, 1 << 16);
      e->release(sl.d_reads);
      sl.d_reads = nullptr;
      sl.cap_bases = 0;
      if ((rc = e->alloc(&sl.d_reads, cb + 16, false))) break;
      sl.cap_bases = cb;
    }
    if (n > sl.cap_reads) {
      const uint64_t cr = std::max<uint64_t>(n, 1024);
      e->release(sl.d_offsets);
      e->release(sl.d_seeds);
      sl.d_offsets = nullptr;
      sl.d_seeds = nullptr;
      sl.cap_reads = 0;
      if ((rc = e->alloc(&sl.d_offsets, cr + 1, false)) || (rc = e->alloc(&sl.d_seeds, cr, false))) break;
      if (sl.h_offsets) (void)hipHostFree(sl.h_offsets);
      if (sl.h_seeds) (void)hipHostFree(sl.h_seeds);
      sl.h_offsets = nullptr;
      sl.h_seeds = nullptr;
      if (!hip_ok(hipHostMalloc(reinterpret_cast<void **>(&sl.h_offsets), (cr + 1) * sizeof(uint64_t), hipHostMallocDefault), "hipHostMalloc") ||
          !hip_ok(hipHostMalloc(reinterpret_cast<void **>(&sl.h_seeds), cr * sizeof(uint32_t), hipHostMallocDefault), "hipHostMalloc"))
        break;
      sl.cap_reads = cr;
    }
    for (uint64_t j = 0; j <= n; ++j) sl.h_offsets[j] = offsets[done + j] - b0;
    memcpy(sl.h_seeds, seeds + done, n * sizeof(uint32_t));
    if (!hip_ok(hipMemcpyAsync(sl.d_reads, reads + b0, bases, hipMemcpyHostToDevice, e->copy_stream), "hipMemcpyAsync(reads)") ||
        !hip_ok(hipMemcpyAsync(sl.d_offsets, sl.h_offsets, (n + 1) * sizeof(uint64_t), hipMemcpyHostToDevice, e->copy_stream), "hipMemcpyAsync(offsets)") ||
        !hip_ok(hipMemcpyAsync(sl.d_seeds, sl.h_seeds, n * sizeof(uint32_t), hipMemcpyHostToDevice, e->copy_stream), "hipMemcpyAsync(seeds)") ||
        !hip_ok(hipEventRecord(sl.copied, e->copy_stream), "hipEventRecord") ||
        !hip_ok(hipStreamWaitEvent(nullptr, sl.copied, 0), "hipStreamWaitEvent"))
      break;
    {
      BatchInput in;
      in.d_reads = sl.d_reads;
      in.d_offsets = sl.d_offsets;
      in.d_seeds = sl.d_seeds;
      in.n_reads = n;
      in.total_bases = bases;
      rc = launch_batch(e, in, nullptr);
    }
    if (rc) break;
    if (!hip_ok(hipEventRecord(sl.done, nullptr), "hipEventRecord")) break;
    sl.busy = true;
    done += n;
  }
  } catch (...) {
    rc = gmx_guard_catch("gmx_map_reads_host");
  }
  (void)hipStreamSynchronize(e->copy_stream);
  (void)hipDeviceSynchronize();
  e->stage[0].busy = e->stage[1].busy = false;
  if (registered) (void)hipHostUnregister(const_cast<uint8_t *>(reads + first));
  (void)hipGetLastError();
  return rc ? rc : gmx_engine_sync(e);
}

static uint64_t gmx_feed_chunk(const gmx_engine *e);
int gmx_map_reads_host(gmx_engine *e, const uint8_t *reads, const uint64_t *offsets, const uint32_t *seeds,
                       uint64_t n_reads) try {
  if (!e) {
    gmx_set_error("null engine");
    return GMX_EINVAL;
  }
  if (n_reads == 0) return GMX_OK;
  HIP_TRY(hipSetDevice(e->opts.device));
  {
    const uint64_t chunk = gmx_feed_chunk(e);
    if (n_reads > chunk && !getenv("GMX_HOST_SERIAL")) return map_reads_host_pipelined(e, reads, offsets, seeds, n_reads, chunk);
  }
  uint64_t done = 0;
  while (done < n_reads) {
    uint64_t n = std::min<uint64_t>(e->opts.max_batch_reads, n_reads - done);
    uint64_t b0 = offsets[done], b1 = offsets[done + n];
    uint64_t bases = b1 - b0;
    if (bases > e->cap_bases) {
      uint64_t cb = std::max<uint64_t>(bases, 1 << 16);
      int rc = e->alloc(&e->d_reads, cb + 16, false);
      if (rc) return rc;
      e->cap_bases = cb;
    }
    if (n > e->cap_stage_reads) {
      uint64_t cr = std::max<uint64_t>(n, 1024);
      int rc = e->alloc(&e->d_offsets, cr + 1, false);
      if (rc) return rc;
      rc = e->alloc(&e->d_seeds, cr, false);
      if (rc) return rc;
      e->cap_stage_reads = cr;
    }
    std::vector<uint64_t> rel(n + 1);
    for (uint64_t i = 0; i <= n; ++i) rel[i] = offsets[done + i] - b0;
    HIP_TRY(hipMemcpy(e->d_reads, reads + b0, bases, hipMemcpyHostToDevice));
    HIP_TRY(hipMemcpy(e->d_offsets, rel.data(), (n + 1) * sizeof(uint64_t), hipMemcpyHostToDevice));
    HIP_TRY(hipMemcpy(e->d_seeds, seeds + done, n * sizeof(uint32_t), hipMemcpyHostToDevice));
    BatchInput in;
    in.d_reads = e->d_reads;
    in.d_offsets = e->d_offsets;
    in.d_seeds = e->d_seeds;
    in.n_reads = n;
    in.total_bases = bases;
    int rc = launch_batch(e, in, nullptr);
    if (rc) return rc;
    HIP_TRY(hipStreamSynchronize(nullptr));
    if (e->log_sites && (rc = log_settle(e))) return rc;
    done += n;
  }
  return gmx_engine_sync(e);
} GMX_GUARD_INT("gmx_map_reads_host")

struct BatchTarget {
  gmx_engine *eng;
  hipStream_t stream;
};
static int pick_target(gmx_engine *e, BatchTarget *out) {
  out->eng = e;
  out->stream = nullptr;
  e->last_on_twin = false;
  gmx_engine *tw = e->twin;
  if (!tw || e->twin_off || e->keep_states) return GMX_OK;
  if (e->reset_pending) {
    e->twin_toggle = 1;
    return GMX_OK;
  }
  if ((e->twin_toggle++ & 1u) == 0) return GMX_OK;
  if (tw->seen_zero_epoch != e->zero_epoch) {
    HIP_TRY(hipStreamWaitEvent(tw->main_stream, e->ev_zeroed, 0));
    tw->seen_zero_epoch = e->zero_epoch;
  }
  tw->timing = e->timing;
  out->eng = tw;
  out->stream = tw->main_stream;
  e->twin_in_flight = true;
  e->last_on_twin = true;
  return GMX_OK;
}

static int map_reads_packed_impl(gmx_engine *e, const uint64_t *planes, bool twobit, const uint64_t *offsets, uint32_t uniform_len,
                                 const uint32_t *seeds, const uint8_t *skip, uint64_t n_reads) {
  if (!e || !planes || !seeds || (!offsets && !uniform_len)) {
    gmx_set_error("gmx_map_reads_packed_host / gmx_map_reads_2bit_host: null argument (offsets may be null only with uniform_len)");
    return GMX_EINVAL;
  }
  if (n_reads == 0) return GMX_OK;
  HIP_TRY(hipSetDevice(e->opts.device));
  if (!e->copy_stream) HIP_TRY(hipStreamCreateWithFlags(&e->copy_stream, hipStreamNonBlocking));
  static const bool two_copy_streams = getenv("GMX_TWO_COPY_STREAMS") != nullptr;
  if (two_copy_streams && !e->copy_stream2) HIP_TRY(hipStreamCreateWithFlags(&e->copy_stream2, hipStreamNonBlocking));
  const uint32_t ppr = (uniform_len + 31u) / 32u;
  auto base_at = [&](uint64_t r) -> uint64_t { return uniform_len ? r * uniform_len : offsets[r] - offsets[0]; };
  auto pair_at = [&](uint64_t r) -> uint64_t {
    if (twobit) return (base_at(r) + 31) >> 5;
    return uniform_len ? r * ppr : ((offsets[r] >> 5) - (offsets[0] >> 5)) + r;
  };
  struct Reg { const void *p; bool on; };
  Reg regs[4] = {{planes, false}, {offsets, false}, {seeds, false}, {skip, false}};
  const uint64_t reg_bytes[4] = {pair_at(n_reads) * 8, (n_reads + 1) * 8, n_reads * 4, n_reads};
  bool all_pinned = true;
  for (int i = 0; i < 4; ++i) {
    if (!regs[i].p || gmx_is_pinned(regs[i].p)) continue;
    regs[i].on = hipHostRegister(const_cast<void *>(regs[i].p), reg_bytes[i], hipHostRegisterDefault) == hipSuccess;
    (void)hipGetLastError();
    all_pinned = false;
  }
  const uint32_t *d_seeds_host = nullptr;
  if (e->seeds_in_place && gmx_is_pinned(seeds)) {
    void *dp = nullptr;
    if (hipHostGetDevicePointer(&dp, const_cast<uint32_t *>(seeds), 0) == hipSuccess && dp) d_seeds_host = static_cast<const uint32_t *>(dp);
    else (void)hipGetLastError();
  }
  const uint64_t chunk = gmx_feed_chunk(e);
  int rc = GMX_OK;
  auto hip_ok = [&](hipError_t err, const char *what) {
    if (err == hipSuccess) return true;
    gmx_set_error(std::string(what) + ": " + hipGetErrorString(err));
    rc = GMX_EHIP;
    return false;
  };
  try {
  for (uint64_t done = 0; done < n_reads && rc == GMX_OK;) {
    gmx_engine::PackSlot &sl = e->pslot[e->pslot_next];
    e->pslot_next = (e->pslot_next + 1) % 3;
    const uint64_t n = std::min<uint64_t>(chunk, n_reads - done);
    uint64_t p0 = pair_at(done), pairs = pair_at(done + n) - p0;
    uint32_t twobit_base0 = 0;
    if (twobit) {
      const uint64_t b0 = base_at(done), b1 = base_at(done + n);
      p0 = b0 >> 5;
      pairs = ((b1 + 31) >> 5) - p0;
      twobit_base0 = (uint32_t)(b0 & 31u);
    }
    if (sl.busy) {
      if (!hip_ok(gmx_event_wait(sl.done), "hipEventSynchronize")) break;
      sl.busy = false;
    }
    if (!sl.copied) {
      if (!hip_ok(hipEventCreateWithFlags(&sl.copied, hipEventDisableTiming | hipEventBlockingSync), "hipEventCreate") ||
          !hip_ok(hipEventCreateWithFlags(&sl.done, hipEventDisableTiming | hipEventBlockingSync), "hipEventCreate"))
        break;
    }
    if (pairs + 16 > sl.cap_pairs) {
      const uint64_t cp = pairs + pairs / 8 + 64;
      e->release(sl.d_planes);
      sl.d_planes = nullptr;
      sl.cap_pairs = 0;
      if ((rc = e->alloc(&sl.d_planes, cp, false))) break;
      sl.cap_pairs = cp;
    }
    if (n > sl.cap_reads) {
      const uint64_t cr = std::max<uint64_t>(n, 1024);
      e->release(sl.d_offsets);
      e->release(sl.d_seeds);
      e->release(sl.d_skip);
      sl.d_offsets = nullptr;
      sl.d_seeds = nullptr;
      sl.d_skip = nullptr;
      sl.cap_reads = 0;
      if ((rc = e->alloc(&sl.d_offsets, cr + 1, false)) || (rc = e->alloc(&sl.d_seeds, cr, false)) || (rc = e->alloc(&sl.d_skip, cr, false))) break;
      sl.cap_reads = cr;
    }
    const hipStream_t cs = two_copy_streams && ((e->copy_toggle++) & 1u) ? e->copy_stream2 : e->copy_stream;
    if (!hip_ok(hipMemcpyAsync(sl.d_planes, planes + p0, pairs * 8, hipMemcpyHostToDevice, cs), "hipMemcpyAsync(planes)")) break;
    if (!uniform_len &&
        !hip_ok(hipMemcpyAsync(sl.d_offsets, offsets + done, (n + 1) * 8, hipMemcpyHostToDevice, cs), "hipMemcpyAsync(offsets)"))
      break;
    if (!d_seeds_host &&
        !hip_ok(hipMemcpyAsync(sl.d_seeds, seeds + done, n * 4, hipMemcpyHostToDevice, cs), "hipMemcpyAsync(seeds)"))
      break;
    if (skip && !hip_ok(hipMemcpyAsync(sl.d_skip, skip + done, n, hipMemcpyHostToDevice, cs), "hipMemcpyAsync(skip)")) break;
    BatchTarget tg;
    if ((rc = pick_target(e, &tg))) break;
    if (!hip_ok(hipEventRecord(sl.copied, cs), "hipEventRecord") ||
        !hip_ok(hipStreamWaitEvent(tg.stream, sl.copied, 0), "hipStreamWaitEvent"))
      break;
    BatchInput in;
    in.d_offsets = uniform_len ? nullptr : sl.d_offsets;
    in.d_seeds = d_seeds_host ? d_seeds_host + done : sl.d_seeds;
    in.d_planes = twobit ? nullptr : sl.d_planes;
    in.d_twobit = twobit ? reinterpret_cast<const uint32_t *>(sl.d_planes) : nullptr;
    in.twobit_base0 = twobit_base0;
    in.d_skip = skip ? sl.d_skip : nullptr;
    in.uniform_len = uniform_len;
    in.n_reads = n;
    in.total_bases = uniform_len ? n * (uint64_t)uniform_len : offsets[done + n] - offsets[done];
    if ((rc = launch_batch(tg.eng, in, tg.stream))) break;
    if (!hip_ok(hipEventRecord(sl.done, tg.stream), "hipEventRecord")) break;
    sl.busy = true;
    done += n;
  }
  } catch (...) {
    rc = gmx_guard_catch(twobit ? "gmx_map_reads_2bit_host" : "gmx_map_reads_packed_host");
  }
  if (rc != GMX_OK || !all_pinned) {
    (void)hipStreamSynchronize(e->copy_stream);
    if (e->copy_stream2) (void)hipStreamSynchronize(e->copy_stream2);
    if (rc != GMX_OK) {
      (void)hipDeviceSynchronize();
      for (auto &sl : e->pslot) sl.busy = false;
    }
  }
  for (int i = 0; i < 4; ++i)
    if (regs[i].on) (void)hipHostUnregister(const_cast<void *>(regs[i].p));
  (void)hipGetLastError();
  return rc;
}

int gmx_map_reads_packed_host(gmx_engine *e, const uint64_t *planes, const uint64_t *offsets, uint32_t uniform_len,
                              const uint32_t *seeds, const uint8_t *skip, uint64_t n_reads) try {
  return map_reads_packed_impl(e, planes, false, offsets, uniform_len, seeds, skip, n_reads);
} GMX_GUARD_INT("gmx_map_reads_packed_host")

static uint64_t gmx_feed_chunk(const gmx_engine *e) {
  static const char *env = getenv("GMX_FEED_CHUNK");
  if (env) return std::max<uint64_t>(1, std::min<uint64_t>(e->opts.max_batch_reads, strtoull(env, nullptr, 10)));
  return e->opts.max_batch_reads;
}

int gmx_map_reads_packed_device(gmx_engine *e, const uint64_t *d_planes, const uint64_t *d_offsets, uint32_t uniform_len,
                                const uint32_t *seeds, const uint8_t *d_skip, uint64_t n_reads) try {
  if (!e || !d_planes || !seeds || (!d_offsets && !uniform_len)) {
    gmx_set_error("gmx_map_reads_packed_device: null argument (d_offsets may be null only with uniform_len)");
    return GMX_EINVAL;
  }
  if (n_reads == 0) return GMX_OK;
  HIP_TRY(hipSetDevice(e->opts.device));
  const uint32_t *d_seeds = seeds;
  if (gmx_is_pinned(seeds)) {
    void *dp = nullptr;
    if (hipHostGetDevicePointer(&dp, const_cast<uint32_t *>(seeds), 0) != hipSuccess || !dp) {
      (void)hipGetLastError();
      gmx_set_error("gmx_map_reads_packed_device: the page-locked seeds have no device address");
      return GMX_EHIP;
    }
    d_seeds = static_cast<const uint32_t *>(dp);
  }
  const uint64_t chunk = gmx_feed_chunk(e);
  if (!uniform_len && n_reads > chunk) {
    gmx_set_error("gmx_map_reads_packed_device: with d_offsets a call takes at most 2^20 reads (and at most max_batch_reads)");
    return GMX_EINVAL;
  }
  const uint64_t ppr = (uniform_len + 31u) / 32u;
  for (uint64_t done = 0; done < n_reads;) {
    const uint64_t n = std::min<uint64_t>(chunk, n_reads - done);
    BatchInput in;
    in.d_planes = reinterpret_cast<const uint2 *>(d_planes + done * ppr);
    in.d_offsets = uniform_len ? nullptr : d_offsets;
    in.d_seeds = d_seeds + done;
    in.d_skip = d_skip ? d_skip + done : nullptr;
    in.uniform_len = uniform_len;
    in.n_reads = n;
    in.total_bases = uniform_len ? n * (uint64_t)uniform_len : 0;
    BatchTarget tg;
    int rc = pick_target(e, &tg);
    if (rc) return rc;
    if ((rc = launch_batch(tg.eng, in, tg.stream))) return rc;
    done += n;
  }
  return GMX_OK;
} GMX_GUARD_INT("gmx_map_reads_packed_device")

int gmx_map_reads_2bit_host(gmx_engine *e, const uint64_t *stream, const uint64_t *offsets, uint32_t uniform_len, const uint32_t *seeds,
                            const uint8_t *skip, uint64_t n_reads) try {
  return map_reads_packed_impl(e, stream, true, offsets, uniform_len, seeds, skip, n_reads);
} GMX_GUARD_INT("gmx_map_reads_2bit_host")

void *gmx_engine_second_stream(gmx_engine *e) { return e && e->twin ? (void *)e->twin->main_stream : nullptr; }

int gmx_engine_seeds_in_place(gmx_engine *e, int on) try {
  if (!e) {
    gmx_set_error("null engine");
    return GMX_EINVAL;
  }
  e->seeds_in_place = on != 0;
  return GMX_OK;
} GMX_GUARD_INT("gmx_engine_seeds_in_place")

int gmx_engine_sync_uploads(gmx_engine *e) try {
  if (!e) {
    gmx_set_error("null engine");
    return GMX_EINVAL;
  }
  HIP_TRY(hipSetDevice(e->opts.device));
  if (e->copy_stream) {
    if (!e->ev_wait) HIP_TRY(hipEventCreateWithFlags(&e->ev_wait, hipEventDisableTiming | hipEventBlockingSync));
    HIP_TRY(hipEventRecord(e->ev_wait, e->copy_stream));
    HIP_TRY(gmx_event_wait(e->ev_wait));
  }
  if (e->copy_stream2) {
    if (!e->ev_wait) HIP_TRY(hipEventCreateWithFlags(&e->ev_wait, hipEventDisableTiming | hipEventBlockingSync));
    HIP_TRY(hipEventRecord(e->ev_wait, e->copy_stream2));
    HIP_TRY(gmx_event_wait(e->ev_wait));
  }
  return GMX_OK;
} GMX_GUARD_INT("gmx_engine_sync_uploads")

static std::mutex g_host_mu;
struct HostBlock {
  uint64_t bytes;
  bool pinned;
};
static std::map<void *, HostBlock> g_host_live;
static std::vector<std::pair<void *, uint64_t>> g_host_spare;
void *gmx_host_alloc(uint64_t bytes) try {
  bytes = std::max<uint64_t>(bytes, 1);
  {
    std::lock_guard<std::mutex> lk(g_host_mu);
    size_t best = g_host_spare.size();
    for (size_t i = 0; i < g_host_spare.size(); ++i)
// ... 33 lines not shown
      g_host_spare.emplace_back(p, blk.bytes);
      return;
    }
  }
  if (blk.pinned)
    (void)hipHostFree(p);
  else
    free(p);
} GMX_GUARD_VOID("gmx_host_free")

int gmx_engine_reserve(gmx_engine *e, uint64_t n_reads, uint64_t n_bases) try {
  if (!e) {
    gmx_set_error("null engine");
    return GMX_EINVAL;
  }
  HIP_TRY(hipSetDevice(e->opts.device));
  n_reads = std::min<uint64_t>(n_reads, e->opts.max_batch_reads);
  int rc = ensure_batch_capacity(e, n_reads);
  if (rc) return rc;
  const uint64_t need = n_bases / 32 + n_reads + 16;
  if (need > e->cap_packed) {
    if ((rc = e->alloc(&e->d_packed, need, false))) return rc;
    e->cap_packed = need;
  }
  if (n_bases > e->cap_bases) {
    if ((rc = e->alloc(&e->d_reads, n_bases + 16, false))) return rc;
    e->cap_bases = n_bases;
  }
  if (n_reads > e->cap_stage_reads) {
    if ((rc = e->alloc(&e->d_offsets, n_reads + 1, false)) || (rc = e->alloc(&e->d_seeds, n_reads, false))) return rc;
    e->cap_stage_reads = n_reads;
  }
  return GMX_OK;
} GMX_GUARD_INT("gmx_engine_reserve")

int gmx_engine_reserve_packed(gmx_engine *e, uint64_t n_reads, uint64_t n_pairs) try {
  if (!e) {
    gmx_set_error("null engine");
    return GMX_EINVAL;
  }
  HIP_TRY(hipSetDevice(e->opts.device));
  n_reads = std::min<uint64_t>(n_reads, gmx_feed_chunk(e));
  int rc = ensure_batch_capacity(e, n_reads);
  if (rc) return rc;
  if (e->twin && (rc = ensure_batch_capacity(e->twin, n_reads))) return rc;
  if (!e->copy_stream) HIP_TRY(hipStreamCreateWithFlags(&e->copy_stream, hipStreamNonBlocking));
  for (auto &sl : e->pslot) {
    if (sl.busy) continue;
    if (!sl.copied) {
      HIP_TRY(hipEventCreateWithFlags(&sl.copied, hipEventDisableTiming | hipEventBlockingSync));
      HIP_TRY(hipEventCreateWithFlags(&sl.done, hipEventDisableTiming | hipEventBlockingSync));
    }
    if (n_pairs + 16 > sl.cap_pairs) {
      e->release(sl.d_planes);
      sl.d_planes = nullptr;
      sl.cap_pairs = 0;
      if ((rc = e->alloc(&sl.d_planes, n_pairs + 64, false))) return rc;
      sl.cap_pairs = n_pairs + 64;
    }
    if (n_reads > sl.cap_reads) {
      e->release(sl.d_offsets);
      e->release(sl.d_seeds);
      e->release(sl.d_skip);
      sl.d_offsets = nullptr;
      sl.d_seeds = nullptr;
      sl.d_skip = nullptr;
      sl.cap_reads = 0;
      if ((rc = e->alloc(&sl.d_offsets, n_reads + 1, false)) || (rc = e->alloc(&sl.d_seeds, n_reads, false)) ||
          (rc = e->alloc(&sl.d_skip, n_reads, false)))
        return rc;
      sl.cap_reads = n_reads;
    }
  }
  return GMX_OK;
} GMX_GUARD_INT("gmx_engine_reserve_packed")

int gmx_engine_sync(gmx_engine *e) try {
  HIP_TRY(hipSetDevice(e->opts.device));
  {
    int frc = flush_reset(e);
    if (frc) return frc;
    if ((frc = log_settle(e))) return frc;
  }
  {
    int qrc = gmx_quiesce(e);
    if (qrc) return qrc;
    if (e->twin && (qrc = gmx_quiesce(e->twin))) return qrc;
    e->twin_in_flight = false;
  }
  HIP_TRY(hipStreamSynchronize(e->last_stream));
  HIP_TRY(hipDeviceSynchronize());
  uint32_t c[4] = {0, 0, 0, 0};
  HIP_TRY(hipMemcpy(c + 2, e->d_error, 8, hipMemcpyDeviceToHost));
  if (c[2] == 0 && e->twin) {
    HIP_TRY(hipMemcpy(c + 2, e->twin->d_error, 8, hipMemcpyDeviceToHost));
    if (c[2] != 0) HIP_TRY(hipMemset(e->twin->d_error, 0, 8));
  }
  if (c[2] != 0) {
    HIP_TRY(hipMemset(e->d_error, 0, 8));
    char msg[256];
    if (c[2] == GMX_TASK_LOGFULL) {
      snprintf(msg, sizeof(msg),
               "a read's records exceed the whole grouped-allele-count log (sites without dense group counters; %u words): "
               "nothing of it was recorded: raise gmx_engine_opts.log_cap_words",
               e->log_cap);
      gmx_set_error(msg);
      return GMX_ECAP;
    }
    if (c[2] == GMX_TASK_OVERFLOW) {
      snprintf(msg, sizeof(msg),
               "read %u (orientation %u) needs more memory for its search states or its mapping instances than the whole "
               "last-tier heap holds (%llu bytes); nothing of this read was recorded: raise gmx_engine_opts.huge_heap_bytes "
               "(GMX_HUGE_HEAP_BYTES)",
               c[3] >> 1, c[3] & 1, (unsigned long long)e->heap_words * 4);
      gmx_set_error(msg);
      return GMX_ECAP;
    }
    snprintf(msg, sizeof(msg),
             "read %u (orientation %u): inconsistent variant path (the reference throws/asserts here: a site "
             "traversed twice or an exit that does not match the entered site)",
             c[3] >> 1, c[3] & 1);
    gmx_set_error(msg);
    return GMX_EREF;
  }
  return GMX_OK;
} GMX_GUARD_INT("gmx_engine_sync")

int gmx_engine_enable_timing(gmx_engine *e, int on) try {
  e->timing = on != 0;
  if (e->twin) e->twin->timing = e->timing;
  return GMX_OK;
} GMX_GUARD_INT("gmx_engine_enable_timing")

int gmx_engine_timing(gmx_engine *e, gmx_timing *out) try {
  HIP_TRY(hipSetDevice(e->opts.device));
  if (e->twin) {
    e->pending.insert(e->pending.end(), e->twin->pending.begin(), e->twin->pending.end());
    e->twin->pending.clear();
  }
  for (auto &ev : e->pending) {
    HIP_TRY(hipEventSynchronize(ev.c));
    float ms0 = 0, ms1 = 0, ms2 = 0;
    HIP_TRY(hipEventElapsedTime(&ms0, ev.s, ev.a));
    HIP_TRY(hipEventElapsedTime(&ms1, ev.a, ev.b));
    HIP_TRY(hipEventElapsedTime(&ms2, ev.b, ev.c));
    e->search_ms += ms1;
    e->cover_ms += ms0 + ms2;
    e->search_launches++;
    e->cover_launches++;
    e->timed_reads += ev.reads;
    for (int k = 0; k < GMX_TK_N; ++k) {
      if (ev.timed & (1u << k)) {
        float ms = 0;
        HIP_TRY(hipEventSynchronize(ev.k[k][1]));
        HIP_TRY(hipEventElapsedTime(&ms, ev.k[k][0], ev.k[k][1]));
        e->kernel_ms[k] += ms;
        e->kernel_launches[k]++;
      }
      (void)hipEventDestroy(ev.k[k][0]);
      (void)hipEventDestroy(ev.k[k][1]);
    }
    (void)hipEventDestroy(ev.s);
    (void)hipEventDestroy(ev.a);
    (void)hipEventDestroy(ev.b);
    (void)hipEventDestroy(ev.c);
  }
  e->pending.clear();
  out->search_ms = e->search_ms;
  out->search_launches = e->search_launches;
  out->cover_ms = e->cover_ms;
  out->cover_launches = e->cover_launches;
  out->reads = e->timed_reads;
  for (int k = 0; k < GMX_TIMED_KERNELS; ++k) {
    out->kernel_ms[k] = e->kernel_ms[k];
    out->kernel_launches[k] = e->kernel_launches[k];
    e->kernel_ms[k] = 0;
    e->kernel_launches[k] = 0;
  }
  e->search_ms = e->cover_ms = 0;
  e->search_launches = e->cover_launches = e->timed_reads = 0;
  return GMX_OK;
} GMX_GUARD_INT("gmx_engine_timing")

int gmx_engine_queue_counts(gmx_engine *e, gmx_queue_counts *out) try {
  HIP_TRY(hipSetDevice(e->opts.device));
  HIP_TRY(hipDeviceSynchronize());
  uint32_t raw[GMX_N_COUNTERS * GMX_CNT_STRIDE];
  HIP_TRY(hipMemcpy(raw, (e->twin && e->last_on_twin ? e->twin : e)->d_counters, sizeof(raw), hipMemcpyDeviceToHost));
  auto c = [&](int i) { return (uint64_t)raw[i * GMX_CNT_STRIDE]; };
  out->mapped = 0;
  for (int r = 0; r < GMX_REGIONS; ++r) out->mapped += c(16 + r);
  out->mapped += c(8);
  out->alive = c(5);
  out->dead = c(6) + c(12);
  out->overflow_probe = c(1);
  out->overflow_extend = c(9);
  out->big_mapped = c(7);
  out->cover_general = c(8);
  out->cover_mid = c(13);
  out->cover_overflow = c(4);
  out->seed_cursor = e->seed_cursor ? 1 : 0;
  out->inst_mapped = c(25);
  out->huge_search = c(11);
  out->huge_cover = c(15);
  out->log_replays = e->log_replays;
  out->log_replayed_entries = e->log_replayed_entries;
  out->overflow_split = c(29);
  return GMX_OK;
} GMX_GUARD_INT("gmx_engine_queue_counts")

int gmx_coverage_device(gmx_engine *e, gmx_device_coverage *out) try {
  {
    int frc = flush_reset(e);
    if (frc) return frc;
  }
  if (e->twin && e->twin_in_flight) {
    int qrc = gmx_quiesce(e->twin);
    if (qrc) return qrc;
    e->twin_in_flight = false;
  }
  out->allele_sum = out->per_base = out->grouped = nullptr;
  out->n_allele_sum = e->n_allele;
  out->n_per_base = e->n_pb;
  out->n_grouped = e->n_grouped;
  out->stats = e->d_stats;
  out->n_stats = 5;
  out->fused = e->d_fused;
  out->n_fused = e->n_fused;
  return GMX_OK;
} GMX_GUARD_INT("gmx_coverage_device")

int gmx_coverage_reduce_begin(gmx_engine *e, void *hip_stream) try {
  if (!e) {
    gmx_set_error("null engine");
    return GMX_EINVAL;
  }
  {
    int frc = flush_reset(e);
    if (frc) return frc;
    if ((frc = log_settle(e))) return frc;
  }
  HIP_TRY(hipSetDevice(e->opts.device));
  {
    int trc = twin_join(e, (hipStream_t)hip_stream);
    if (trc) return trc;
  }
  e->recorded = true;
  hipLaunchKernelGGL(gmx_stats_limbs_kernel, dim3(1), dim3(64), 0, (hipStream_t)hip_stream, e->d_stats, e->d_limbs, 0);
  HIP_TRY(hipGetLastError());
  return GMX_OK;
} GMX_GUARD_INT("gmx_coverage_reduce_begin")

int gmx_coverage_reduce_end(gmx_engine *e, void *hip_stream) try {
  if (!e) {
    gmx_set_error("null engine");
    return GMX_EINVAL;
  }
  {
    int frc = flush_reset(e);
    if (frc) return frc;
  }
  HIP_TRY(hipSetDevice(e->opts.device));
  hipLaunchKernelGGL(gmx_stats_limbs_kernel, dim3(1), dim3(64), 0, (hipStream_t)hip_stream, e->d_stats, e->d_limbs, 1);
  HIP_TRY(hipGetLastError());
  return GMX_OK;
} GMX_GUARD_INT("gmx_coverage_reduce_end")

static void gather_block(const gmx_engine *e, const uint32_t *block, uint32_t *allele_sum, uint32_t *per_base, uint32_t *grouped) {
  if (allele_sum) for (size_t i = 0; i < e->phys_allele.size(); ++i) allele_sum[i] += block[e->phys_allele[i]];
  if (per_base) for (size_t i = 0; i < e->phys_pb.size(); ++i) per_base[i] += block[e->phys_pb[i]];
  if (grouped) for (size_t i = 0; i < e->phys_grouped.size(); ++i) grouped[i] += block[e->phys_grouped[i]];
  for (size_t i = 0; i + 3 < e->hit_fix.size(); i += 4) {
    const uint32_t hits = block[e->hit_fix[i]];
    if (allele_sum) allele_sum[e->hit_fix[i + 1]] += hits;
    if (grouped) grouped[e->hit_fix[i + 2]] += hits;
    if (per_base) per_base[e->hit_fix[i + 3]] += hits;
  }
}
static int fetch_blocks(gmx_engine *e, size_t first, size_t count, uint32_t *allele_sum, uint32_t *per_base, uint32_t *grouped) {
  {
    int frc = flush_reset(e);
    if (frc) return frc;
    if ((frc = log_settle(e))) return frc;
  }
  HIP_TRY(hipSetDevice(e->opts.device));
  HIP_TRY(hipDeviceSynchronize());
  if (!allele_sum && !per_base && !grouped) return GMX_OK;
  std::vector<uint32_t> block(std::max<size_t>(e->n_acc * count, 1));
  if (e->n_acc) HIP_TRY(hipMemcpy(block.data(), e->d_fused + first * e->n_acc, e->n_acc * count * 4, hipMemcpyDeviceToHost));
  if (allele_sum) std::fill(allele_sum, allele_sum + e->phys_allele.size(), 0u);
  if (per_base) std::fill(per_base, per_base + e->phys_pb.size(), 0u);
  if (grouped) std::fill(grouped, grouped + e->phys_grouped.size(), 0u);
  for (size_t k = 0; k < count; ++k) gather_block(e, block.data() + k * e->n_acc, allele_sum, per_base, grouped);
  return GMX_OK;
}

int gmx_coverage_fetch(gmx_engine *e, uint32_t *allele_sum, uint32_t *per_base, uint32_t *grouped, gmx_stats *stats) try {
  if (!e) {
    gmx_set_error("null engine");
    return GMX_EINVAL;
  }
  {
    int rc = fetch_blocks(e, 0, e->record_strands ? 2 : 1, allele_sum, per_base, grouped);
    if (rc) return rc;
  }
  if (stats) {
    unsigned long long s[5];
    HIP_TRY(hipMemcpy(s, e->d_stats, sizeof(s), hipMemcpyDeviceToHost));
    stats->all_reads_count = s[0];
    stats->skipped_reads_count = s[1];
    stats->missing_kmer_reads_count = s[2];
    stats->no_extension_reads_count = s[3];
    stats->exact_mapped_reads_count = s[4];
  }
  return GMX_OK;
} GMX_GUARD_INT("gmx_coverage_fetch")

int gmx_coverage_fetch_strand(gmx_engine *e, int strand, uint32_t *allele_sum, uint32_t *per_base, uint32_t *grouped_dense) try {
  if (!e) {
    gmx_set_error("null engine");
    return GMX_EINVAL;
  }
  if (!e->record_strands) {
    gmx_set_error("gmx_coverage_fetch_strand: the engine does not record per strand (gmx_engine_record_strands)");
    return GMX_EINVAL;
  }
  if (strand != 0 && strand != 1) {
    gmx_set_error("gmx_coverage_fetch_strand: strand is 0 (forward) or 1 (reverse complement)");
    return GMX_EINVAL;
  }
  return fetch_blocks(e, (size_t)strand, 1, allele_sum, per_base, grouped_dense);
} GMX_GUARD_INT("gmx_coverage_fetch_strand")

static int set_record_strands(gmx_engine *e, bool on) {
  if (e->record_strands == on) return GMX_OK;
  const size_t n_fused = (on ? 2 : 1) * e->n_acc + 32;
  if (n_fused + 32 > 0xFFFFFFFFull) {
    gmx_set_error("gmx_engine_record_strands: two accumulator blocks of this index exceed 2^32 words");
    return GMX_EINVAL;
  }
  uint32_t *old = e->d_fused, *q = nullptr;
  int rc = e->alloc(&q, n_fused + 32, true);
  if (rc) return rc;
  e->release(old);
  e->record_strands = on;
  e->reset_pending = false;
  for (gmx_engine *w : {e, e->twin}) {
    if (!w) continue;
    w->d_fused = q;
    w->n_fused = n_fused;
    w->d_limbs = q + n_fused - 32;
    w->d_stats = reinterpret_cast<unsigned long long *>(q + n_fused);
    w->d_log_cursor = q + n_fused + 16;
  }
  return GMX_OK;
}

int gmx_engine_record_strands(gmx_engine *e, int on) try {
  if (!e) {
    gmx_set_error("null engine");
    return GMX_EINVAL;
  }
  if (e->recorded) {
    gmx_set_error("gmx_engine_record_strands: coverage has been recorded since the last reset (call gmx_engine_reset first)");
    return GMX_EINVAL;
  }
  HIP_TRY(hipSetDevice(e->opts.device));
  HIP_TRY(hipDeviceSynchronize());
  return set_record_strands(e, on != 0);
} GMX_GUARD_INT("gmx_engine_record_strands")

int gmx_engine_set_max_candidates(gmx_engine *e, uint32_t limit) try {
  if (!e) {
    gmx_set_error("null engine");
    return GMX_EINVAL;
  }
  if (e->recorded) {
    gmx_set_error("gmx_engine_set_max_candidates: coverage has been recorded since the last reset (call gmx_engine_reset first)");
    return GMX_EINVAL;
  }
  e->max_candidates = limit;
  return GMX_OK;
} GMX_GUARD_INT("gmx_engine_set_max_candidates")

uint32_t gmx_engine_max_candidates(gmx_engine *e) try {
  return e ? e->max_candidates : 0u;
} GMX_GUARD_ZERO("gmx_engine_max_candidates")

static int read_log_record(gmx_engine *e, GmxReadLog gmx_engine::*log, int on) {
  if (!e) {
    gmx_set_error("null engine");
    return GMX_EINVAL;
  }
  (e->*log).on = on != 0;
  return GMX_OK;
}

static int64_t read_log_count(gmx_engine *e, GmxReadLog gmx_engine::*log) {
  if (!e) {
    gmx_set_error("null engine");
    return GMX_EINVAL;
  }
  return (int64_t)(e->*log).count;
}

static int read_log_fetch(gmx_engine *e, GmxReadLog gmx_engine::*which, uint64_t first, uint64_t n, void *out, const char *name) {
  if (!e || (n && !out)) {
    gmx_set_error(std::string(name) + ": null argument");
    return GMX_EINVAL;
  }
  const GmxReadLog &log = e->*which;
  if (first > log.count || n > log.count - first) {
    gmx_set_error(std::string(name) + ": reads " + std::to_string(first) + " .. " + std::to_string(first + n) + " of " +
                  std::to_string(log.count) + " recorded");
    return GMX_EINVAL;
  }
  {
    int frc = flush_reset(e);
// ... 29 lines not shown
      if (!count) continue;
      if (out && n + words <= cap_words) {
        out[n] = kv.first[0];
        out[n + 1] = (uint32_t)(kv.first.size() - 1) | GMX_LOG_COUNTED | (which == LOG_EXCHANGE && s ? GMX_LOG_REVERSE : 0u);
        out[n + 2] = (uint32_t)count;
        out[n + 3] = (uint32_t)(count >> 32);
        for (size_t j = 1; j < kv.first.size(); ++j) out[n + 3 + j] = kv.first[j];
      }
      n += words;
    }
  }
  return n;
}

int gmx_engine_record_positions(gmx_engine *e, int on) try {
  return read_log_record(e, &gmx_engine::positions, on);
} GMX_GUARD_INT("gmx_engine_record_positions")

int64_t gmx_engine_position_count(gmx_engine *e) try {
  return read_log_count(e, &gmx_engine::positions);
} GMX_GUARD_INT("gmx_engine_position_count")

int gmx_engine_fetch_positions(gmx_engine *e, uint64_t first, uint64_t n, uint32_t *out) try {
  return read_log_fetch(e, &gmx_engine::positions, first, n, out, "gmx_engine_fetch_positions");
} GMX_GUARD_INT("gmx_engine_fetch_positions")

int64_t gmx_coverage_fetch_grouped_log(gmx_engine *e, uint32_t *out, uint64_t cap_words) try {
  if (!e) return GMX_EINVAL;
  if (hipSetDevice(e->opts.device) != hipSuccess) return GMX_EHIP;
  if (log_settle(e)) return GMX_EHIP;
  if (gmx_log_drain(e, 0)) return GMX_EHIP;
  return (int64_t)emit_log_counts(e, LOG_TOTALS, out, cap_words);
} GMX_GUARD_INT("gmx_coverage_fetch_grouped_log")

int64_t gmx_coverage_fetch_grouped_log_strand(gmx_engine *e, int strand, uint32_t *out, uint64_t cap_words) try {
  if (!e) {
    gmx_set_error("null engine");
    return GMX_EINVAL;
  }
  if (!e->record_strands) {
    gmx_set_error("gmx_coverage_fetch_grouped_log_strand: the engine does not record per strand (gmx_engine_record_strands)");
    return GMX_EINVAL;
  }
  if (strand != 0 && strand != 1) {
    gmx_set_error("gmx_coverage_fetch_grouped_log_strand: strand is 0 (forward) or 1 (reverse complement)");
    return GMX_EINVAL;
  }
  if (hipSetDevice(e->opts.device) != hipSuccess) return GMX_EHIP;
  if (log_settle(e)) return GMX_EHIP;
  if (gmx_log_drain(e, 0)) return GMX_EHIP;
  return (int64_t)emit_log_counts(e, strand ? LOG_REVERSE_ONLY : LOG_FORWARD, out, cap_words);
} GMX_GUARD_INT("gmx_coverage_fetch_grouped_log_strand")

int64_t gmx_coverage_export_grouped_log(gmx_engine *e, uint32_t *out, uint64_t cap_words) try {
  if (!e) {
    gmx_set_error("null engine");
    return GMX_EINVAL;
  }
  if (hipSetDevice(e->opts.device) != hipSuccess) return GMX_EHIP;
  if (log_settle(e)) return GMX_EHIP;
  if (gmx_log_drain(e, 0)) return GMX_EHIP;
  return (int64_t)emit_log_counts(e, exchange_form(e), out, cap_words);
} GMX_GUARD_INT("gmx_coverage_export_grouped_log")

int gmx_coverage_import_grouped_log(gmx_engine *e, const uint32_t *records, uint64_t n_words, int replace) try {
  if (!e || (!records && n_words)) {
    gmx_set_error("gmx_coverage_import_grouped_log: null argument");
    return GMX_EINVAL;
  }
  {
    int frc = flush_reset(e);
    if (frc) return frc;
  }
  HIP_TRY(hipSetDevice(e->opts.device));
  return gmx_engine_log_import(e, records, (size_t)n_words, replace != 0);
} GMX_GUARD_INT("gmx_coverage_import_grouped_log")

}

uint64_t gmx_engine_reset_epoch(const gmx_engine *e) { return e->reset_epoch; }

void gmx_engine_raw(gmx_engine *e, GmxEngineRaw *out) {
  (void)flush_reset(e);
  out->device = e->opts.device;
  out->d_fused = e->d_fused;
  out->n_fused = e->n_fused;
  out->log_sites = e->log_sites;
  out->record_strands = e->record_strands;
}

int gmx_engine_log_export(gmx_engine *e, std::vector<uint32_t> &out) {
  {
    int frc = flush_reset(e);
    if (frc) return frc;
    if ((frc = log_settle(e))) return frc;
  }
  HIP_TRY(hipSetDevice(e->opts.device));
  {
    int rc = gmx_log_drain(e, 0);
    if (rc) return rc;
  }
  const LogForm which = exchange_form(e);
  out.assign((size_t)emit_log_counts(e, which, nullptr, 0), 0);
  emit_log_counts(e, which, out.data(), out.size());
  return GMX_OK;
}

int gmx_engine_log_import(gmx_engine *e, const uint32_t *w, size_t n_words, bool replace) {
  {
    int frc = flush_reset(e);
    if (frc) return frc;
  }
  const uint32_t flags = GMX_LOG_COUNTED | GMX_LOG_REVERSE;
  for (size_t i = 0; i < n_words;) {
    if (w[i] == GMX_LOG_PAD) {
      ++i;
      continue;
    }
    if (i + 2 > n_words) break;
    const uint32_t n = w[i + 1] & ~flags;
    const size_t head = (w[i + 1] & GMX_LOG_COUNTED) ? 4 : 2;
    if (i + head + n > n_words) {
      gmx_set_error("corrupt grouped log");
      return GMX_EINVAL;
    }
    if ((w[i + 1] & GMX_LOG_REVERSE) && !e->record_strands) {
      gmx_set_error("grouped log: a reverse-complement record (GMX_LOG_REVERSE) for an engine that does not record per strand");
      return GMX_EINVAL;
    }
    i += head + n;
  }
  if (replace) {
    int rc = gmx_log_drain(e, 0);
    if (rc) return rc;
    e->log_counts.clear();
  }
  std::vector<uint32_t> key;
  for (size_t i = 0; i < n_words;) {
    if (w[i] == GMX_LOG_PAD) {
      ++i;
      continue;
    }
    if (i + 2 > n_words) break;
    const uint32_t n = w[i + 1] & ~flags;
    const size_t head = (w[i + 1] & GMX_LOG_COUNTED) ? 4 : 2;
    const uint64_t count = head == 4 ? ((uint64_t)w[i + 2] | ((uint64_t)w[i + 3] << 32)) : 1;
    key.assign(1, w[i]);
    key.insert(key.end(), w + i + head, w + i + head + n);
    e->log_counts[key][(w[i + 1] & GMX_LOG_REVERSE) ? 1 : 0] += count;
    i += head + n;
  }
  return GMX_OK;
}

#include "gmx_engine_debug.h"
```

### gramtools_amd/csrc/gmx_index.cpp

```cpp
#include "gmx_index.h"

#include <algorithm>
#include <array>
#include <limits>
#include <atomic>
#include <chrono>
#include <cstdio>
#include <functional>
#include <memory>
#include <cstring>
#include <fstream>
#include <sys/stat.h>
#include <map>
#include <mutex>
#include <stdexcept>
#include <thread>
#include <unordered_map>

#include "gmx_core.h"
#include "gmx_internal.h"

namespace gmx {

namespace {
// ... 1831 lines not shown
    w.pod(h.n_seed_states);
    w.pod(h.n_seed_states_large);
    index_tables(w, h);
    w.pod<uint64_t>(h.target_map.size());
    for (auto const &e : h.target_map) {
      w.pod(e.first);
      w.vec(e.second);
    }
    w.pod<uint64_t>(w.sum.value());
    w.pod(kCacheMagic);
  } catch (...) {
    fclose(f);
    remove(tmp.c_str());
    throw;
  }
  if (fclose(f) != 0 || rename(tmp.c_str(), path.c_str()) != 0) {
    remove(tmp.c_str());
    throw std::runtime_error("index cache: cannot finish " + path);
  }
}

void load_index(const std::string &path, const std::vector<uint32_t> &prg, uint32_t kmer_size, HostIndex &out) {
  FILE *f = fopen(path.c_str(), "rb");
  if (!f) throw std::runtime_error("index cache: cannot open " + path);
  try {
    Reader r{f};
    {
      struct stat st;
      if (fstat(fileno(f), &st) == 0 && st.st_size >= 0) r.left = (uint64_t)st.st_size;
    }
    uint64_t magic = 0, n_prg = 0, hash = 0;
    uint32_t version = 0, nested = 0;
    r.pod(magic);
    r.pod(version);
    if (magic != kCacheMagic || version != kCacheVersion) throw std::runtime_error("index cache: not a version-" + std::to_string(kCacheVersion) + " cache file");
    r.pod(n_prg);
    r.pod(hash);
    r.pod(out.kmer_size);
    r.pod(out.kmer_size2);
    r.pod(out.seed_shift);
    if (out.seed_shift > 8) throw std::runtime_error("index cache: corrupt header");
    if (n_prg != prg.size() || hash != fnv1a_u32(prg)) throw std::runtime_error("index cache: built from a different PRG");
    if (out.kmer_size != kmer_size) throw std::runtime_error("index cache: built for a different kmer_size");
    r.pod(out.sentinel_pos);
    r.raw(out.C, sizeof(out.C));
    r.pod(nested);
    out.is_nested = nested != 0;
    r.pod(out.n_allele_slots);
    r.pod(out.n_pb_slots);
    r.pod(out.n_grouped_slots);
    r.pod(out.n_acc_slots);
    r.pod(out.n_seed_kmers_present);
    r.pod(out.n_seed_states);
    r.pod(out.n_seed_states_large);
    index_tables(r, out);
    uint64_t n_tm = 0;
    r.pod(n_tm);
    if (n_tm > prg.size() + 1) throw std::runtime_error("index cache: implausible table size");
    out.target_map.resize(n_tm);
    for (auto &e : out.target_map) {
      r.pod(e.first);
      r.vec(e.second);
    }
    const uint64_t computed = r.sum.value();
    uint64_t stored = 0, end = 0;
    r.pod(stored);
    r.pod(end);
    if (end != kCacheMagic || stored != computed) throw std::runtime_error("index cache: damaged file (checksum)");
    out.prg = prg;
    if (out.sa.size() != prg.size() + 1 || out.pos_node.size() != prg.size() || out.text.size() != prg.size() / 64 + 1 ||
        out.seeds.size() != (kmer_size ? (1ull << (2 * kmer_size)) : 0) ||
        out.seeds2.size() != (out.kmer_size2 ? (1ull << (2 * out.kmer_size2)) : 0) || out.kmer_size2 > 15 || out.nodes.empty() || out.phys_allele.size() != out.n_allele_slots ||
        out.phys_pb.size() != out.n_pb_slots || out.phys_grouped.size() != out.n_grouped_slots || out.hit_fix.size() % 4 != 0 || out.site_ref_pos.size() != out.sites.size() ||
        out.site_geo.size() != out.sites.size() ||
        (out.seed_words.size() >> out.seed_shift) >= (1ull << 30))
      throw std::runtime_error("index cache: inconsistent tables");
  } catch (...) {
    fclose(f);
    throw;
  }
  fclose(f);
}

}
```

### gramtools_amd/csrc/gmx_index.h

```cpp
#pragma once
#include <sys/mman.h>

#include <algorithm>
#include <chrono>
#include <cstdint>
#include <cstdlib>
#include <new>
#include <string>
#include <utility>
#include <vector>

#include "gmx_types.h"

namespace gmx {

inline bool gmx_huge_pages_pay() {
  static const bool ok = [] {
    if (const char *e = getenv("GMX_HUGEPAGES")) return atoi(e) != 0;
    const size_t bytes = (size_t)16 << 20, huge = (size_t)2 << 20;
    auto touch = [&](bool advise) -> double {
      void *p = aligned_alloc(huge, bytes);
      if (!p) return 1e9;
      if (advise && madvise(p, bytes, MADV_HUGEPAGE) != 0) {
        free(p);
// ... 97 lines not shown
struct TargetedMarker {
  uint32_t id;
  int32_t deletion_allele;
};

struct HostIndex {
  std::vector<uint32_t> prg;
  uint32_t kmer_size = 0;
  uint32_t sentinel_pos = 0;
  uint32_t C[8] = {0};
  bool is_nested = false;

  std::vector<GmxRankBlock> blocks;
  std::vector<uint32_t> sa;
  std::vector<GmxHit> hits;
  std::vector<uint32_t> hit_perm, hit_prog;
  std::vector<GmxTextRec> text;
  std::vector<uint32_t> prog;
  std::vector<uint32_t> pos_node;
  std::vector<GmxNode> nodes;
  std::vector<uint32_t> edges;
  std::vector<GmxSite> sites;
  std::vector<GmxSiteGeo> site_geo;
  SeedTable seeds;
  uint32_t kmer_size2 = 0;
  SeedTable seeds2;
  WordBuf seed_words;
  uint32_t seed_shift = 0;
  std::vector<uint32_t> kmer_bitmap;
  uint32_t n_allele_slots = 0, n_pb_slots = 0, n_grouped_slots = 0;
  uint32_t n_acc_slots = 0;
  std::vector<uint32_t> l_allele_off, l_grouped_off;
  std::vector<uint32_t> l_cov_off;
  std::vector<uint32_t> phys_allele, phys_pb, phys_grouped;
  std::vector<uint32_t> hit_fix;
  std::vector<uint32_t> site_ref_pos;

  std::vector<uint32_t> bwt;
  std::vector<std::pair<uint32_t, std::vector<TargetedMarker>>> target_map;
  std::vector<std::pair<uint32_t, int32_t>> pos_target;
  uint64_t n_seed_kmers_present = 0;
  uint64_t n_seed_states = 0, n_seed_states_large = 0;

  GmxIndexView view() const;
};

void build_suffix_array(const std::vector<uint32_t> &text, std::vector<uint32_t> &sa, int threads = 1);
void debug_suffix_array_u16(const uint16_t *text, size_t n, uint16_t *sa);

void build_index(const std::vector<uint32_t> &prg, uint32_t kmer_size, HostIndex &out, int threads = 0, int seed_k2 = -1);
void build_index(std::vector<uint32_t> &&prg, uint32_t kmer_size, HostIndex &out, int threads = 0, int seed_k2 = -1);

void save_index(const HostIndex &h, const std::string &path);
void load_index(const std::string &path, const std::vector<uint32_t> &prg, uint32_t kmer_size, HostIndex &out);

std::vector<uint32_t> read_prg_file(const std::string &path);

struct WalkState {
  uint32_t lo, hi, tvd, tvg;
};
struct WalkNode {
  std::vector<WalkState> list;
  std::vector<GmxPathNode> arena;
};
struct SeedEntryRef {
  uint32_t code, table;
  uint64_t off;
};
struct SeedPart {
  std::vector<uint32_t> words;
  uint64_t word_base = 0, n_words = 0;
  std::vector<SeedEntryRef> complex;
  uint64_t n_present[2] = {0, 0}, n_states_all[2] = {0, 0}, n_states_large[2] = {0, 0};
};
typedef bool (*DeviceSeedWalk)(const HostIndex &ix, uint32_t k, uint32_t k2, uint32_t depth0, std::vector<WalkNode> &roots,
                               GmxSeed *table, GmxSeed *table2, uint32_t *bitmap, std::vector<SeedPart> &parts, WordBuf &words);
extern DeviceSeedWalk g_device_seed_walk;

typedef bool (*DeviceSuffixPresort)(const uint32_t *text, size_t n, uint32_t *sa, std::vector<uint32_t> &tie_mask);
extern DeviceSuffixPresort g_device_suffix_presort;

std::vector<int64_t> seed_states_of(const HostIndex &ix, uint32_t kmer_code, bool longer_table = false);

}
```

### include/gmx.h

```cpp
#ifndef GMX_H
#define GMX_H
#include <stddef.h>
#include <stdint.h>

#ifdef __cplusplus
extern "C" {
#endif

#define GMX_OK 0
#define GMX_EINVAL (-1)
#define GMX_ENODEV (-2)
#define GMX_EHIP (-3)
#define GMX_ECAP (-4)
#define GMX_EREF (-5)
#define GMX_ENOMEM (-6)

typedef struct gmx_index gmx_index;
typedef struct gmx_engine gmx_engine;

const char *gmx_last_error(void);

int gmx_index_build(const uint32_t *prg, uint64_t n_symbols, uint32_t kmer_size, int threads, gmx_index **out);
int gmx_index_build_from_file(const char *prg_path, uint32_t kmer_size, int threads, gmx_index **out);
int gmx_index_save(const gmx_index *ix, const char *path);
int gmx_index_load(const char *cache_path, const char *prg_path, uint32_t kmer_size, gmx_index **out);
void gmx_index_destroy(gmx_index *ix);

typedef struct gmx_index_info {
  uint64_t n_text;
  uint32_t kmer_size;
  uint32_t n_sites;
  uint32_t is_nested;
  uint32_t n_allele_slots;
  uint32_t n_per_base_slots;
  uint32_t n_grouped_slots;
  uint32_t n_nodes;
  uint64_t n_kmers_present;
  uint64_t index_bytes;
  uint32_t kmer_size2;
  uint32_t n_inline_sites;
  uint32_t seed_shift;
  uint32_t n_jump_sites;
  uint64_t n_seed_words;
} gmx_index_info;
int gmx_index_get_info(const gmx_index *ix, gmx_index_info *out);

int gmx_index_site_layout(const gmx_index *ix, uint32_t *n_alleles, uint32_t *allele_sum_off, uint32_t *grouped_off,
                          uint32_t *parent_site, int32_t *parent_allele);
int64_t gmx_index_per_base_layout(const gmx_index *ix, uint32_t *out, uint64_t cap_records);
int gmx_index_allele_base_layout(const gmx_index *ix, uint32_t *pb_off, uint32_t *len);

typedef struct gmx_depth_stats {
  double mean_cov_depth, variance_cov_depth;
  uint64_t num_sites_noCov, num_sites_total;
} gmx_depth_stats;
int gmx_compute_coverage_depth(const gmx_index *ix, const uint32_t *per_base_raw, const uint32_t *grouped_dense_raw,
                               const uint32_t *grouped_log, uint64_t n_log_words, gmx_depth_stats *out);
int gmx_index_bubble_order(const gmx_index *ix, uint32_t *site_markers_out);

int gmx_debug_suffix_array_u16(const uint16_t *text, uint64_t n, uint16_t *out);
int gmx_index_copy_sa(const gmx_index *ix, uint32_t *out);
int gmx_index_copy_bwt(const gmx_index *ix, uint32_t *out);
uint32_t gmx_index_rank(const gmx_index *ix, uint32_t upper, uint32_t base);
int gmx_index_copy_pos_info(const gmx_index *ix, int64_t *out);
int64_t gmx_index_copy_target_map(const gmx_index *ix, int64_t *out, uint64_t cap);
int64_t gmx_index_seed_states(const gmx_index *ix, const uint8_t *kmer, int64_t *out, uint64_t cap);
int64_t gmx_index_seed_states_k(const gmx_index *ix, const uint8_t *kmer, uint32_t len, int64_t *out, uint64_t cap);
int64_t gmx_index_jump_states(const gmx_index *ix, uint32_t lo, uint32_t hi, int64_t *out, uint64_t cap);

typedef struct gmx_engine_opts {
  int device;
  int rng_mode;
  uint32_t max_states;
  uint32_t max_path_nodes;
  uint64_t max_batch_reads;
  int forward_only;
  uint64_t huge_heap_bytes;
  uint64_t log_cap_words;
} gmx_engine_opts;
void gmx_engine_default_opts(gmx_engine_opts *opts);

int gmx_engine_create(const gmx_index *ix, const gmx_engine_opts *opts, gmx_engine **out);
void gmx_engine_destroy(gmx_engine *e);
int gmx_engine_reset(gmx_engine *e);
int gmx_engine_reset_async(gmx_engine *e, void *hip_stream);

int gmx_map_reads_host(gmx_engine *e, const uint8_t *reads, const uint64_t *offsets, const uint32_t *seeds,
                       uint64_t n_reads);
int gmx_map_reads_device(gmx_engine *e, const uint8_t *d_reads, const uint64_t *d_offsets, const uint32_t *d_seeds,
                         uint64_t n_reads, uint64_t total_bases, void *hip_stream);
int gmx_map_reads_packed_host(gmx_engine *e, const uint64_t *planes, const uint64_t *offsets, uint32_t uniform_len,
                              const uint32_t *seeds, const uint8_t *skip, uint64_t n_reads);
int gmx_engine_sync_uploads(gmx_engine *e);
int gmx_engine_seeds_in_place(gmx_engine *e, int on);
uint64_t gmx_packed_pairs(const uint64_t *offsets, uint32_t uniform_len, uint64_t n_reads);
int gmx_pack_reads(const uint8_t *reads, const uint64_t *offsets, uint32_t uniform_len, uint64_t n_reads, uint64_t *planes,
                   uint8_t *skip, int threads);
int gmx_map_reads_2bit_host(gmx_engine *e, const uint64_t *stream, const uint64_t *offsets, uint32_t uniform_len,
                            const uint32_t *seeds, const uint8_t *skip, uint64_t n_reads);
uint64_t gmx_twobit_units(const uint64_t *offsets, uint32_t uniform_len, uint64_t n_reads);
int gmx_pack_reads_2bit(const uint8_t *reads, const uint64_t *offsets, uint32_t uniform_len, uint64_t n_reads, uint64_t *stream,
                        uint8_t *skip, int threads);
int gmx_map_reads_packed_device(gmx_engine *e, const uint64_t *d_planes, const uint64_t *d_offsets, uint32_t uniform_len,
                                const uint32_t *seeds, const uint8_t *d_skip, uint64_t n_reads);
void *gmx_engine_second_stream(gmx_engine *e);

typedef struct gmx_ingest gmx_ingest;
typedef struct {
  uint64_t offset;
  uint32_t size;
  uint32_t isize;
  uint32_t crc32;
  uint32_t reserved;
} gmx_bgzf_member;
#define GMX_INGEST_BAD_RECORD 1u
#define GMX_INGEST_BAD_MEMBER 2u
#define GMX_INGEST_BAD_CRC 4u
#define GMX_INGEST_TOO_MANY_LINES 8u
#define GMX_INGEST_GZ_UNREPAIRED 16u
#define GMX_INGEST_GZ_LOOKAHEAD 32u
#define GMX_INGEST_GZ_PIECE_BOUND 64u
#define GMX_INGEST_GZ_MEMBER_ENDS 128u
#define GMX_INGEST_GZ_TEXT_LIMIT 256u
typedef struct {
  uint32_t status;
  uint32_t bad_member;
  uint64_t n_reads, n_bases, n_pairs;
  uint32_t uniform_len;
  uint32_t any_skip;
  uint64_t text_bytes;
  uint64_t consumed_bytes, tail_bytes;
  uint64_t sub_pairs[16];
  const uint64_t *d_planes, *d_offsets;
  const uint8_t *d_skip;
} gmx_ingest_result;
int gmx_ingest_create(int device, uint64_t max_text_bytes, gmx_ingest **out);
void gmx_ingest_destroy(gmx_ingest *g);
uint64_t gmx_ingest_max_text(const gmx_ingest *g);
uint64_t gmx_ingest_max_compressed(const gmx_ingest *g);
uint64_t gmx_ingest_max_members(const gmx_ingest *g);
int gmx_ingest_reset(gmx_ingest *g);
#define GMX_INGEST_FORMAT_FASTQ 0
#define GMX_INGEST_FORMAT_FASTA 1
// ... 194 lines not shown
```

Baseline: 1.453 billion.

## Gather coverage on device and skip redundant syncs when engine is idle

Moves the coverage gather (fused accumulator to allele/per-base/grouped arrays, including hit fixups) from a host loop to a GPU kernel driven by precomputed inverse index maps. The stats and error/retry counters are packed into a trailer and copied back in one async transfer into pinned memory. An idle/scattered/exposed tracking scheme lets later log drains and quiesce calls skip device-wide synchronization when nothing has run since a clean fetch. The idle tracking depends on every mutating path calling gmx_touch, so a missed call site could skip required synchronization.

```diff
diff --git a/gramtools_amd/_lib.py b/gramtools_amd/_lib.py
--- a/gramtools_amd/_lib.py
+++ b/gramtools_amd/_lib.py
@@ -87,6 +87,7 @@
     "gmx_compute_coverage_depth": (C.c_int, [_vp, _u32p, _u32p, _u32p, _u64, C.POINTER(DepthStats)]),
     "gmx_index_bubble_order": (C.c_int, [_vp, _u32p]),
     "gmx_debug_suffix_array_u16": (C.c_int, [C.POINTER(C.c_uint16), _u64, C.POINTER(C.c_uint16)]),
+    "gmx_debug_gather_maps": (C.c_int, [_u32p, _u64, _u32p, _u64, _u32p, _u64, _u32p, _u64, _u64, _u32p, _u32p]),
     "gmx_index_copy_sa": (C.c_int, [_vp, _u32p]),
     "gmx_index_copy_bwt": (C.c_int, [_vp, _u32p]),
     "gmx_index_rank": (_u32, [_vp, _u32, _u32]),
diff --git a/gramtools_amd/csrc/gmx_capi.cpp b/gramtools_amd/csrc/gmx_capi.cpp
--- a/gramtools_amd/csrc/gmx_capi.cpp
+++ b/gramtools_amd/csrc/gmx_capi.cpp
@@ -426,6 +426,25 @@
   }
 } GMX_GUARD_INT("gmx_debug_suffix_array_u16")
 
+int gmx_debug_gather_maps(const uint32_t *phys_allele, uint64_t n_allele, const uint32_t *phys_pb, uint64_t n_pb, const uint32_t *phys_grouped,
+                          uint64_t n_grouped, const uint32_t *hit_fix, uint64_t n_hit_words, uint64_t n_acc, uint32_t *word, uint32_t *hit) try {
+  if ((n_allele && !phys_allele) || (n_pb && !phys_pb) || (n_grouped && !phys_grouped) || (n_hit_words && !hit_fix) ||
+      ((n_allele + n_pb + n_grouped) && (!word || !hit))) {
+    gmx_set_error("gmx_debug_gather_maps: null argument");
+    return GMX_EINVAL;
+  }
+  std::vector<uint32_t> w, h;
+  if (!gmx::invert_gather_maps(std::vector<uint32_t>(phys_allele, phys_allele + n_allele), std::vector<uint32_t>(phys_pb, phys_pb + n_pb),
+                               std::vector<uint32_t>(phys_grouped, phys_grouped + n_grouped), std::vector<uint32_t>(hit_fix, hit_fix + n_hit_words),
+                               n_acc, w, h))
+    return 0;
+  if (!w.empty()) {
+    memcpy(word, w.data(), w.size() * 4);
+    memcpy(hit, h.data(), h.size() * 4);
+  }
+  return 1;
+} GMX_GUARD_INT("gmx_debug_gather_maps")
+
 int gmx_index_copy_sa(const gmx_index *ix, uint32_t *out) try {
   memcpy(out, ix->h.sa.data(), ix->h.sa.size() * 4);
   return GMX_OK;
diff --git a/gramtools_amd/csrc/gmx_engine_cover_kernels.h b/gramtools_amd/csrc/gmx_engine_cover_kernels.h
--- a/gramtools_amd/csrc/gmx_engine_cover_kernels.h
+++ b/gramtools_amd/csrc/gmx_engine_cover_kernels.h
@@ -893,6 +893,40 @@
   }
 }
 
+#define GMX_GATHER_TRAILER 32u
+#define GMX_GATHER_THREADS 256
+struct GatherTrailerSrc {
+  const unsigned long long *stats;
+  const uint32_t *log_cursor, *counters, *error, *twin_error;
+};
+__global__ void __launch_bounds__(GMX_GATHER_THREADS) gmx_gather_kernel(const uint32_t *block, uint64_t n_acc, uint32_t n_blocks, const uint32_t *word,
+                                                                        const uint32_t *hit, uint32_t n_slots, uint32_t *out, uint64_t trailer_at,
+                                                                        GatherTrailerSrc src) {
+  const uint64_t i = (uint64_t)blockIdx.x * GMX_GATHER_THREADS + threadIdx.x;
+  if (i < n_slots) {
+    const uint32_t w = word[i], h = hit[i];
+    uint32_t v = 0;
+    for (uint32_t k = 0; k < n_blocks; ++k) {
+      const uint32_t *b = block + k * n_acc;
+      v += b[w];
+      if (h != GMX_GATHER_NO_HIT) v += b[h];
+    }
+    out[i] = v;
+  }
+  if (blockIdx.x == 0 && threadIdx.x < GMX_GATHER_TRAILER) {
+    const uint32_t t = threadIdx.x;
+    uint32_t v = 0;
+    if (t < 10) v = (uint32_t)(src.stats[t >> 1] >> (32 * (t & 1)));
+    else if (t == 10) v = src.log_cursor[0];
+    else if (t == 11) v = src.counters[GMX_CNT_LOG_RETRY * GMX_CNT_STRIDE];
+    else if (t == 12) v = src.counters[GMX_CNT_LOG_RETRY_RECS * GMX_CNT_STRIDE];
+    else if (t == 13) v = src.counters[GMX_CNT_LOG_RETRY_HUGE * GMX_CNT_STRIDE];
+    else if (t < 16) v = src.error[t - 14];
+    else if (t < 18) v = src.twin_error ? src.twin_error[t - 16] : 0u;
+    out[trailer_at + t] = v;
+  }
+}
+
 #define GMX_PACK_READS 128
 #define GMX_PACK_IN_BYTES (24 * 1024)
 #define GMX_PACK_OUT_PAIRS (GMX_PACK_IN_BYTES / 32 + GMX_PACK_READS + 8)
diff --git a/gramtools_amd/csrc/gmx_engine_debug.h b/gramtools_amd/csrc/gmx_engine_debug.h
--- a/gramtools_amd/csrc/gmx_engine_debug.h
+++ b/gramtools_amd/csrc/gmx_engine_debug.h
@@ -198,6 +198,7 @@
     return GMX_EINVAL;
   }
   HIP_TRY(hipSetDevice(e->opts.device));
+  gmx_touch(e);
   HIP_TRY(hipDeviceSynchronize());
   int rc = debug_isa(e);
   if (rc) return rc;
@@ -307,6 +308,7 @@
     return GMX_EINVAL;
   }
   HIP_TRY(hipSetDevice(e->opts.device));
+  gmx_touch(e);
   HIP_TRY(hipDeviceSynchronize());
   int rc = debug_isa(e);
   if (rc) return rc;
@@ -377,6 +379,7 @@
     return GMX_EINVAL;
   }
   HIP_TRY(hipSetDevice(e->opts.device));
+  gmx_touch(e);
   HIP_TRY(hipDeviceSynchronize());
   std::vector<GmxFinalState> st;
   std::vector<GmxPathNode> arena;
diff --git a/gramtools_amd/csrc/gmx_engine_host.h b/gramtools_amd/csrc/gmx_engine_host.h
--- a/gramtools_amd/csrc/gmx_engine_host.h
+++ b/gramtools_amd/csrc/gmx_engine_host.h
@@ -178,6 +178,17 @@
     bool busy = false;
   } pslot[3];
   uint32_t pslot_next = 0;
+  struct Fetch {
+    int state = 0;
+    uint32_t *d_word = nullptr, *d_hit = nullptr, *d_out = nullptr, *h_out = nullptr;
+    uint64_t n_slots = 0;
+    hipEvent_t ev = nullptr;
+  } fetch;
+  bool fetch_host_gather = false;
+  bool scattered = false;
+  bool exposed = false;
+  bool idle = false;
+  uint32_t idle_cursor = 0;
   void release(void *q) {
     if (!q) return;
     for (size_t i = 0; i < allocs.size(); ++i)
@@ -276,9 +287,16 @@
   HIP_TRY(hipStreamWaitEvent(stream, e->ev_twin_done, 0));
   return GMX_OK;
 }
+static void gmx_touch(gmx_engine *e) { (e->owner ? e->owner : e)->idle = false; }
+static void gmx_touch(gmx_engine *e, hipStream_t stream) {
+  gmx_engine *own = e->owner ? e->owner : e;
+  own->idle = false;
+  if (stream != own->last_stream) own->scattered = true;
+}
 static int flush_reset(gmx_engine *e) {
   if (!e->reset_pending) return GMX_OK;
   e->reset_pending = false;
+  gmx_touch(e, e->reset_stream);
   HIP_TRY(hipMemsetAsync(e->d_fused, 0, (e->n_fused + 32) * 4, e->reset_stream));
   return note_zeroed(e, e->reset_stream);
 }
@@ -287,6 +305,11 @@
 static int gmx_log_drain(gmx_engine *e, uint64_t keep_below) {
   int frc = flush_reset(e);
   if (frc) return frc;
+  if (e->idle && e->idle_cursor == 0) {
+    e->log_reads_since = 0;
+    e->log_known = 0;
+    return GMX_OK;
+  }
   HIP_TRY(hipDeviceSynchronize());
   uint32_t used = 0;
   HIP_TRY(hipMemcpy(&used, e->d_log_cursor, 4, hipMemcpyDeviceToHost));
@@ -294,6 +317,7 @@
   e->log_reads_since = 0;
   e->log_known = used;
   if (used <= keep_below) return GMX_OK;
+  gmx_touch(e);
   std::vector<uint32_t> w(used);
   HIP_TRY(hipMemcpy(w.data(), e->d_log, (size_t)used * 4, hipMemcpyDeviceToHost));
   std::vector<uint32_t> key;
@@ -353,6 +377,7 @@
 } GMX_GUARD_VOID("gmx_engine_default_opts")
 
 static int ensure_batch_capacity(gmx_engine *e, uint64_t n_reads, bool launching = false) {
+  gmx_touch(e);
   if (launching) {
     gmx_engine *own = e->owner ? e->owner : e;
     for (GmxReadLog *log : {&own->outcomes, &own->positions})
@@ -672,6 +697,7 @@
     }
   }
   if (getenv("GMX_NO_COOP")) e->coop = false;
+  if (const char *hg = getenv("GMX_FETCH_HOST_GATHER")) e->fetch_host_gather = atoi(hg) != 0;
   e->seed_cursor = h.n_seed_states_large * 10 > h.n_seed_states;
   if (const char *sc = getenv("GMX_SEED_CURSOR")) e->seed_cursor = atoi(sc) != 0;
   if (primary) {
@@ -759,6 +785,8 @@
   if (e->copy_stream2) (void)hipStreamDestroy(e->copy_stream2);
   if (e->h_log_state) (void)hipHostFree(e->h_log_state);
   if (e->ev_log_state) (void)hipEventDestroy(e->ev_log_state);
+  if (e->fetch.ev) (void)hipEventDestroy(e->fetch.ev);
+  if (e->fetch.h_out) gmx_host_free(e->fetch.h_out);
   for (auto &sl : e->pslot) {
     if (sl.copied) (void)hipEventDestroy(sl.copied);
     if (sl.done) (void)hipEventDestroy(sl.done);
@@ -779,6 +807,7 @@
 int gmx_engine_reset(gmx_engine *e) try {
   HIP_TRY(hipSetDevice(e->opts.device));
   e->reset_pending = false;
+  gmx_touch(e, nullptr);
   HIP_TRY(hipDeviceSynchronize());
   HIP_TRY(hipMemset(e->d_fused, 0, (e->n_fused + 32) * 4));
   HIP_TRY(hipMemset(e->d_error, 0, 8));
@@ -803,6 +832,7 @@
   hipStream_t st = (hipStream_t)hip_stream;
   int frc = flush_reset(e);
   if (frc) return frc;
+  gmx_touch(e, st);
   if ((frc = twin_join(e, st))) return frc;
   e->twin_in_flight = false;
   if ((frc = e->outcomes.clear(&st)) || (frc = e->positions.clear(&st))) return frc;
@@ -833,6 +863,7 @@
 }
 
 static int log_state_enqueue(gmx_engine *e, hipStream_t stream) {
+  gmx_touch(e);
   if (!e->h_log_state) {
     HIP_TRY(hipHostMalloc(reinterpret_cast<void **>(&e->h_log_state), 4 * sizeof(uint32_t), hipHostMallocDefault));
     HIP_TRY(hipEventCreateWithFlags(&e->ev_log_state, hipEventDisableTiming));
@@ -848,6 +879,7 @@
 
 static int launch_log_replay(gmx_engine *e, hipStream_t stream) {
   const int in = e->log_retry_side, out = in ^ 1;
+  gmx_touch(e);
   SearchOut o = e->last_o;
   o.log_retry_list = e->d_log_retry[out];
   o.log_retry_recs = e->d_log_retry_recs[out];
@@ -884,6 +916,7 @@
       return GMX_OK;
     }
     if (round > 0 && retries >= before) {
+      gmx_touch(e);
       HIP_TRY(hipDeviceSynchronize());
       const uint32_t err[2] = {GMX_TASK_LOGFULL, 0};
       HIP_TRY(hipMemcpy(e->d_error, err, 8, hipMemcpyHostToDevice));
@@ -961,6 +994,8 @@
 static int launch_batch(gmx_engine *e, const BatchInput &in, hipStream_t stream) {
   const uint64_t n_reads = in.n_reads, total_bases = in.total_bases;
   if (n_reads == 0) return GMX_OK;
+  if (e->is_twin) gmx_touch(e);
+  else gmx_touch(e, stream);
   if (n_reads > (0x7fffffffull / GMX_FAST_ARENA) / 2) {
     gmx_set_error("batch too large: at most 44 M reads per launch (lower gmx_engine_opts.max_batch_reads)");
     return GMX_EINVAL;
@@ -1238,6 +1273,7 @@
 
 static int map_reads_host_pipelined(gmx_engine *e, const uint8_t *reads, const uint64_t *offsets, const uint32_t *seeds,
                                     uint64_t n_reads, uint64_t chunk) {
+  gmx_touch(e);
   if (!e->copy_stream) HIP_TRY(hipStreamCreateWithFlags(&e->copy_stream, hipStreamNonBlocking));
   const uint64_t first = offsets[0], total = offsets[n_reads] - first;
   const bool registered = !gmx_is_pinned(reads + first) &&
@@ -1332,6 +1368,7 @@
   }
   if (n_reads == 0) return GMX_OK;
   HIP_TRY(hipSetDevice(e->opts.device));
+  gmx_touch(e);
   {
     const uint64_t chunk = gmx_feed_chunk(e);
     if (n_reads > chunk && !getenv("GMX_HOST_SERIAL")) return map_reads_host_pipelined(e, reads, offsets, seeds, n_reads, chunk);
@@ -1410,6 +1447,7 @@
   }
   if (n_reads == 0) return GMX_OK;
   HIP_TRY(hipSetDevice(e->opts.device));
+  gmx_touch(e);
   if (!e->copy_stream) HIP_TRY(hipStreamCreateWithFlags(&e->copy_stream, hipStreamNonBlocking));
   static const bool two_copy_streams = getenv("GMX_TWO_COPY_STREAMS") != nullptr;
   if (two_copy_streams && !e->copy_stream2) HIP_TRY(hipStreamCreateWithFlags(&e->copy_stream2, hipStreamNonBlocking));
@@ -1550,6 +1588,7 @@
   }
   if (n_reads == 0) return GMX_OK;
   HIP_TRY(hipSetDevice(e->opts.device));
+  gmx_touch(e);
   const uint32_t *d_seeds = seeds;
   if (gmx_is_pinned(seeds)) {
     void *dp = nullptr;
@@ -1749,6 +1788,10 @@
     if (frc) return frc;
     if ((frc = log_settle(e))) return frc;
   }
+  if (e->idle) {
+    e->twin_in_flight = false;
+    return GMX_OK;
+  }
   {
     int qrc = gmx_quiesce(e);
     if (qrc) return qrc;
@@ -1757,6 +1800,7 @@
   }
   HIP_TRY(hipStreamSynchronize(e->last_stream));
   HIP_TRY(hipDeviceSynchronize());
+  e->scattered = false;
   uint32_t c[4] = {0, 0, 0, 0};
   HIP_TRY(hipMemcpy(c + 2, e->d_error, 8, hipMemcpyDeviceToHost));
   if (c[2] == 0 && e->twin) {
@@ -1886,6 +1930,8 @@
     if (qrc) return qrc;
     e->twin_in_flight = false;
   }
+  gmx_touch(e);
+  e->exposed = true;
   out->allele_sum = out->per_base = out->grouped = nullptr;
   out->n_allele_sum = e->n_allele;
   out->n_per_base = e->n_pb;
@@ -1913,6 +1959,7 @@
     if (trc) return trc;
   }
   e->recorded = true;
+  gmx_touch(e, (hipStream_t)hip_stream);
   hipLaunchKernelGGL(gmx_stats_limbs_kernel, dim3(1), dim3(64), 0, (hipStream_t)hip_stream, e->d_stats, e->d_limbs, 0);
   HIP_TRY(hipGetLastError());
   return GMX_OK;
@@ -1928,6 +1975,7 @@
     if (frc) return frc;
   }
   HIP_TRY(hipSetDevice(e->opts.device));
+  gmx_touch(e, (hipStream_t)hip_stream);
   hipLaunchKernelGGL(gmx_stats_limbs_kernel, dim3(1), dim3(64), 0, (hipStream_t)hip_stream, e->d_stats, e->d_limbs, 1);
   HIP_TRY(hipGetLastError());
   return GMX_OK;
@@ -1944,21 +1992,116 @@
     if (per_base) per_base[e->hit_fix[i + 3]] += hits;
   }
 }
-static int fetch_blocks(gmx_engine *e, size_t first, size_t count, uint32_t *allele_sum, uint32_t *per_base, uint32_t *grouped) {
+static void stats_from_words(const uint32_t *w, gmx_stats *stats) {
+  auto u64 = [&](int i) { return (uint64_t)w[2 * i] | ((uint64_t)w[2 * i + 1] << 32); };
+  stats->all_reads_count = u64(0);
+  stats->skipped_reads_count = u64(1);
+  stats->missing_kmer_reads_count = u64(2);
+  stats->no_extension_reads_count = u64(3);
+  stats->exact_mapped_reads_count = u64(4);
+}
+static int fetch_blocks_host(gmx_engine *e, size_t first, size_t count, uint32_t *allele_sum, uint32_t *per_base, uint32_t *grouped, gmx_stats *stats) {
+  HIP_TRY(hipDeviceSynchronize());
+  e->scattered = false;
+  if (allele_sum || per_base || grouped) {
+    std::vector<uint32_t> block(std::max<size_t>(e->n_acc * count, 1));
+    if (e->n_acc) HIP_TRY(hipMemcpy(block.data(), e->d_fused + first * e->n_acc, e->n_acc * count * 4, hipMemcpyDeviceToHost));
+    if (allele_sum) std::fill(allele_sum, allele_sum + e->phys_allele.size(), 0u);
+    if (per_base) std::fill(per_base, per_base + e->phys_pb.size(), 0u);
+    if (grouped) std::fill(grouped, grouped + e->phys_grouped.size(), 0u);
+    for (size_t k = 0; k < count; ++k) gather_block(e, block.data() + k * e->n_acc, allele_sum, per_base, grouped);
+  }
+  if (stats) {
+    uint32_t s[10];
+    HIP_TRY(hipMemcpy(s, e->d_stats, sizeof(s), hipMemcpyDeviceToHost));
+    stats_from_words(s, stats);
+  }
+  return GMX_OK;
+}
+static bool fetch_setup(gmx_engine *e) {
+  gmx_engine::Fetch &f = e->fetch;
+  if (f.state) return f.state > 0;
+  if (e->fetch_host_gather) {
+    f.state = -1;
+    return false;
+  }
+  std::vector<uint32_t> word, hit;
+  if (!gmx::invert_gather_maps(e->phys_allele, e->phys_pb, e->phys_grouped, e->hit_fix, e->n_acc, word, hit)) {
+    f.state = -1;
+    return false;
+  }
+  e->allocs.reserve(e->allocs.size() + 3);
+  const uint64_t n = word.size();
+  uint32_t *dw = nullptr, *dh = nullptr, *dout = nullptr, *h = nullptr;
+  hipEvent_t ev = nullptr;
+  bool ok = e->alloc(&dw, n, false) == GMX_OK && e->alloc(&dh, n, false) == GMX_OK && e->alloc(&dout, n + GMX_GATHER_TRAILER, false) == GMX_OK;
+  if (ok && n)
+    ok = hipMemcpy(dw, word.data(), n * 4, hipMemcpyHostToDevice) == hipSuccess && hipMemcpy(dh, hit.data(), n * 4, hipMemcpyHostToDevice) == hipSuccess;
+  if (ok) {
+    h = static_cast<uint32_t *>(gmx_host_alloc((n + GMX_GATHER_TRAILER) * 4));
+    ok = h && gmx_is_pinned(h);
+  }
+  if (ok) ok = hipEventCreateWithFlags(&ev, hipEventDisableTiming) == hipSuccess;
+  if (!ok) {
+    (void)hipGetLastError();
+    if (h) gmx_host_free(h);
+    e->release(dw);
+    e->release(dh);
+    e->release(dout);
+    f.state = -1;
+    return false;
+  }
+  f.d_word = dw;
+  f.d_hit = dh;
+  f.d_out = dout;
+  f.h_out = h;
+  f.n_slots = n;
+  f.ev = ev;
+  f.state = 1;
+  return true;
+}
+static int fetch_blocks(gmx_engine *e, size_t first, size_t count, uint32_t *allele_sum, uint32_t *per_base, uint32_t *grouped, gmx_stats *stats) {
   {
     int frc = flush_reset(e);
     if (frc) return frc;
     if ((frc = log_settle(e))) return frc;
   }
   HIP_TRY(hipSetDevice(e->opts.device));
-  HIP_TRY(hipDeviceSynchronize());
-  if (!allele_sum && !per_base && !grouped) return GMX_OK;
-  std::vector<uint32_t> block(std::max<size_t>(e->n_acc * count, 1));
-  if (e->n_acc) HIP_TRY(hipMemcpy(block.data(), e->d_fused + first * e->n_acc, e->n_acc * count * 4, hipMemcpyDeviceToHost));
-  if (allele_sum) std::fill(allele_sum, allele_sum + e->phys_allele.size(), 0u);
-  if (per_base) std::fill(per_base, per_base + e->phys_pb.size(), 0u);
-  if (grouped) std::fill(grouped, grouped + e->phys_grouped.size(), 0u);
-  for (size_t k = 0; k < count; ++k) gather_block(e, block.data() + k * e->n_acc, allele_sum, per_base, grouped);
+  if (!fetch_setup(e)) return fetch_blocks_host(e, first, count, allele_sum, per_base, grouped, stats);
+  gmx_engine::Fetch &f = e->fetch;
+  const bool arrays = allele_sum || per_base || grouped;
+  std::vector<uint32_t> trailer(GMX_GATHER_TRAILER);
+  hipStream_t st = e->last_stream;
+  if (e->scattered || e->exposed) {
+    HIP_TRY(hipDeviceSynchronize());
+    e->scattered = false;
+  } else {
+    int trc = twin_join(e, st);
+    if (trc) return trc;
+  }
+  const uint32_t n = arrays ? (uint32_t)f.n_slots : 0u;
+  const GatherTrailerSrc src{e->d_stats, e->d_log_cursor, e->d_counters, e->d_error, e->twin ? e->twin->d_error : nullptr};
+  hipLaunchKernelGGL(gmx_gather_kernel, dim3(std::max<uint32_t>((n + GMX_GATHER_THREADS - 1) / GMX_GATHER_THREADS, 1u)), dim3(GMX_GATHER_THREADS), 0, st,
+                     e->d_fused + first * e->n_acc, (uint64_t)e->n_acc, (uint32_t)count, f.d_word, f.d_hit, n, f.d_out, f.n_slots, src);
+  HIP_TRY(hipGetLastError());
+  const size_t from = arrays ? 0 : (size_t)f.n_slots;
+  HIP_TRY(hipMemcpyAsync(f.h_out + from, f.d_out + from, ((size_t)f.n_slots + GMX_GATHER_TRAILER - from) * 4, hipMemcpyDeviceToHost, st));
+  HIP_TRY(hipEventRecord(f.ev, st));
+  HIP_TRY(hipEventSynchronize(f.ev));
+  const size_t na = e->phys_allele.size(), np = e->phys_pb.size(), ng = e->phys_grouped.size();
+  if (allele_sum && na) memcpy(allele_sum, f.h_out, na * 4);
+  if (per_base && np) memcpy(per_base, f.h_out + na, np * 4);
+  if (grouped && ng) memcpy(grouped, f.h_out + na + np, ng * 4);
+  std::copy(f.h_out + f.n_slots, f.h_out + f.n_slots + GMX_GATHER_TRAILER, trailer.begin());
+  const uint32_t *t = trailer.data();
+  if (stats) stats_from_words(t, stats);
+  bool clean = !e->exposed;
+  for (int i = 11; i < 18; ++i) clean = clean && t[i] == 0;
+  e->idle = clean;
+  if (clean) {
+    e->idle_cursor = t[10];
+    e->twin_in_flight = false;
+  }
   return GMX_OK;
 }
 
@@ -1967,20 +2110,7 @@
     gmx_set_error("null engine");
     return GMX_EINVAL;
   }
-  {
-    int rc = fetch_blocks(e, 0, e->record_strands ? 2 : 1, allele_sum, per_base, grouped);
-    if (rc) return rc;
-  }
-  if (stats) {
-    unsigned long long s[5];
-    HIP_TRY(hipMemcpy(s, e->d_stats, sizeof(s), hipMemcpyDeviceToHost));
-    stats->all_reads_count = s[0];
-    stats->skipped_reads_count = s[1];
-    stats->missing_kmer_reads_count = s[2];
-    stats->no_extension_reads_count = s[3];
-    stats->exact_mapped_reads_count = s[4];
-  }
-  return GMX_OK;
+  return fetch_blocks(e, 0, e->record_strands ? 2 : 1, allele_sum, per_base, grouped, stats);
 } GMX_GUARD_INT("gmx_coverage_fetch")
 
 int gmx_coverage_fetch_strand(gmx_engine *e, int strand, uint32_t *allele_sum, uint32_t *per_base, uint32_t *grouped_dense) try {
@@ -1996,11 +2126,12 @@
     gmx_set_error("gmx_coverage_fetch_strand: strand is 0 (forward) or 1 (reverse complement)");
     return GMX_EINVAL;
   }
-  return fetch_blocks(e, (size_t)strand, 1, allele_sum, per_base, grouped_dense);
+  return fetch_blocks(e, (size_t)strand, 1, allele_sum, per_base, grouped_dense, nullptr);
 } GMX_GUARD_INT("gmx_coverage_fetch_strand")
 
 static int set_record_strands(gmx_engine *e, bool on) {
   if (e->record_strands == on) return GMX_OK;
+  gmx_touch(e);
   const size_t n_fused = (on ? 2 : 1) * e->n_acc + 32;
   if (n_fused + 32 > 0xFFFFFFFFull) {
     gmx_set_error("gmx_engine_record_strands: two accumulator blocks of this index exceed 2^32 words");
@@ -2196,6 +2327,8 @@
 
 void gmx_engine_raw(gmx_engine *e, GmxEngineRaw *out) {
   (void)flush_reset(e);
+  gmx_touch(e);
+  e->exposed = true;
   out->device = e->opts.device;
   out->d_fused = e->d_fused;
   out->n_fused = e->n_fused;
diff --git a/gramtools_amd/csrc/gmx_index.cpp b/gramtools_amd/csrc/gmx_index.cpp
--- a/gramtools_amd/csrc/gmx_index.cpp
+++ b/gramtools_amd/csrc/gmx_index.cpp
@@ -1937,4 +1937,28 @@
   fclose(f);
 }
 
-}
+bool invert_gather_maps(const std::vector<uint32_t> &phys_allele, const std::vector<uint32_t> &phys_pb, const std::vector<uint32_t> &phys_grouped,
+                        const std::vector<uint32_t> &hit_fix, uint64_t n_acc, std::vector<uint32_t> &word, std::vector<uint32_t> &hit) {
+  const uint64_t na = phys_allele.size(), np = phys_pb.size(), ng = phys_grouped.size(), total = na + np + ng;
+  if (total >= GMX_GATHER_NO_HIT || hit_fix.size() % 4 != 0) return false;
+  word.clear();
+  word.reserve(total);
+  word.insert(word.end(), phys_allele.begin(), phys_allele.end());
+  word.insert(word.end(), phys_pb.begin(), phys_pb.end());
+  word.insert(word.end(), phys_grouped.begin(), phys_grouped.end());
+  for (uint32_t w : word)
+    if (w >= n_acc) return false;
+  hit.assign(total, GMX_GATHER_NO_HIT);
+  for (size_t i = 0; i < hit_fix.size(); i += 4) {
+    const uint32_t counter = hit_fix[i];
+    if (counter >= n_acc || hit_fix[i + 1] >= na || hit_fix[i + 2] >= ng || hit_fix[i + 3] >= np) return false;
+    const uint64_t slots[3] = {hit_fix[i + 1], na + hit_fix[i + 3], na + np + hit_fix[i + 2]};
+    for (uint64_t s : slots) {
+      if (hit[s] != GMX_GATHER_NO_HIT) return false;
+      hit[s] = counter;
+    }
+  }
+  return true;
+}
+
+}
diff --git a/gramtools_amd/csrc/gmx_index.h b/gramtools_amd/csrc/gmx_index.h
--- a/gramtools_amd/csrc/gmx_index.h
+++ b/gramtools_amd/csrc/gmx_index.h
@@ -203,4 +203,8 @@
 
 std::vector<int64_t> seed_states_of(const HostIndex &ix, uint32_t kmer_code, bool longer_table = false);
 
+#define GMX_GATHER_NO_HIT 0xFFFFFFFFu
+bool invert_gather_maps(const std::vector<uint32_t> &phys_allele, const std::vector<uint32_t> &phys_pb, const std::vector<uint32_t> &phys_grouped,
+                        const std::vector<uint32_t> &hit_fix, uint64_t n_acc, std::vector<uint32_t> &word, std::vector<uint32_t> &hit);
+
 }
diff --git a/include/gmx.h b/include/gmx.h
--- a/include/gmx.h
+++ b/include/gmx.h
@@ -59,6 +59,8 @@
 int gmx_index_bubble_order(const gmx_index *ix, uint32_t *site_markers_out);
 
 int gmx_debug_suffix_array_u16(const uint16_t *text, uint64_t n, uint16_t *out);
+int gmx_debug_gather_maps(const uint32_t *phys_allele, uint64_t n_allele, const uint32_t *phys_pb, uint64_t n_pb, const uint32_t *phys_grouped,
+                          uint64_t n_grouped, const uint32_t *hit_fix, uint64_t n_hit_words, uint64_t n_acc, uint32_t *word, uint32_t *hit);
 int gmx_index_copy_sa(const gmx_index *ix, uint32_t *out);
 int gmx_index_copy_bwt(const gmx_index *ix, uint32_t *out);
 uint32_t gmx_index_rank(const gmx_index *ix, uint32_t upper, uint32_t base);
```

Result: no change. 1.452 billion (median of 2 runs) (-0.0%).
